# placrosse/Zaru

Hardware: AMD Instinct MI355X
Metric: end-to-end faces/sec (detect+468-pt mesh), 1080p synthetic, 1/2/4/8 GPU (higher is better)
Workload: dtype f32

## Files before the change

include/zaru_hip.h:

```cpp
#ifndef ZARU_HIP_H
#define ZARU_HIP_H

#include <stddef.h>
#include <stdint.h>

#ifdef __cplusplus
extern "C" {
#endif

#define ZR_OK 0
#define ZR_ERR_INVALID_ARGUMENT (-1)
#define ZR_ERR_MODEL (-2)
#define ZR_ERR_DEVICE (-3)
#define ZR_ERR_SHAPE (-4)
#define ZR_ERR_INTERNAL (-5)

typedef struct zr_session zr_session;

typedef struct {
    float cx, cy, w, h, rad;
} zr_view;

typedef struct {
    const uint8_t *rgba;
// ... 41 lines not shown
    int mode;
} zr_detpost_cfg;
int zr_detect_post_async(const float *d_logits, const float *d_boxes, const float *d_anchors,
                         const float *d_letterbox, size_t n, const zr_detpost_cfg *cfg,
                         int32_t *d_count, float *d_dets, size_t dcap, float *d_records, size_t rmax,
                         uint32_t first_id, uint32_t id_stride, int32_t *d_ties, void *hip_stream);

int zr_detect_post_mapped_async(const float *d_logits, const float *d_boxes, const float *d_anchors,
                                const float *d_letterbox, size_t n, const int32_t *d_map, const int32_t *d_nframes,
                                const zr_detpost_cfg *cfg, int32_t *d_count, float *d_dets, size_t dcap,
                                int32_t *d_ties, void *hip_stream);

typedef struct {
    int tiles, tile_cap;
    int keypoints;
    float iou;
    int mode;
} zr_detmerge_cfg;
int zr_detect_merge_async(const int32_t *d_tile_count, const float *d_tile_dets, const int32_t *d_due,
                          const int32_t *d_ndue, size_t n, const zr_detmerge_cfg *cfg, int32_t *d_count,
                          float *d_dets, size_t dcap, int32_t *d_ties, int32_t *d_tile_dropped, void *hip_stream);

int zr_embed_match_async(const float *d_query, size_t q, const float *d_gallery, size_t g, size_t dim,
                         const int32_t *d_valid, int32_t *d_best_idx, float *d_best_dist,
                         float *d_dist , void *hip_stream);
int zr_embed_match_count_async(const float *d_query, size_t q, const float *d_gallery, size_t g_cap,
                               const int32_t *d_g, size_t dim, const int32_t *d_valid, int32_t *d_best_idx,
                               float *d_best_dist, void *hip_stream);

typedef struct zr_comm zr_comm;
int zr_comm_unique_id(uint8_t id[128]);
int zr_comm_create(const uint8_t id[128], int nranks, int rank, int device, zr_comm **out);
void zr_comm_destroy(zr_comm *c);
int zr_comm_size(const zr_comm *c, int *nranks);
int zr_comm_all_gather_async(zr_comm *c, const void *d_send, void *d_recv, size_t bytes, void *hip_stream);

typedef struct {
    float roi[5];
    float view_rect[5];
    float local[3];
    uint32_t active;
    uint32_t frame_w, frame_h;
    uint32_t tracked;
    float confidence;
    float updated[5];
} zr_track_state;

typedef struct {
    float half_w, half_h, tl_x, tl_y, view_w, view_h, cos_r, sin_r;
    uint32_t frame, pad;
} zr_view_desc;

typedef struct {
    int kind;
    int num_landmarks;
    int in_w, in_h;
    int aspect_w, aspect_h;
    float loss_thresh, padding;
    int rois_per_frame;
} zr_track_cfg;

int zr_track_seed_async(zr_track_state *d_state, size_t n, const zr_track_cfg *cfg,
                        zr_view_desc *d_views, void *hip_stream);
int zr_track_update_async(zr_track_state *d_state, size_t n, const zr_track_cfg *cfg,
                          const float *d_landmarks, size_t lm_stride, const float *d_flag,
                          size_t flag_stride, float *d_lm_out, zr_view_desc *d_views, void *hip_stream);
int zr_track_update_indexed_async(zr_track_state *d_state, size_t n, const zr_track_cfg *cfg,
                                  const float *d_landmarks, size_t lm_stride, const float *d_flag,
                                  size_t flag_stride, const int32_t *d_index, float *d_lm_out,
                                  zr_view_desc *d_views, void *hip_stream);

enum { ZR_LM_FILTER_NONE = 0, ZR_LM_FILTER_EMA = 1, ZR_LM_FILTER_ALPHA_BETA = 2, ZR_LM_FILTER_ONE_EURO = 3 };
typedef struct {
    int kind;
    float p[3];
} zr_lm_filter;
int zr_lm_filter_state_size(const zr_lm_filter *filter, size_t num_landmarks, size_t *bytes);
int zr_lm_filter_async(const zr_lm_filter *filter, const zr_track_cfg *cfg, const zr_track_state *d_state,
                       size_t n, const float *d_landmarks, size_t lm_stride, const float *d_flag,
                       size_t flag_stride, float elapsed_s, void *d_filter_state, float *d_positions,
                       void *hip_stream);
int zr_track_update_positions_async(zr_track_state *d_state, size_t n, const zr_track_cfg *cfg,
                                    const float *d_positions, const float *d_flag, size_t flag_stride,
                                    float *d_lm_out, zr_view_desc *d_views, void *hip_stream);
int zr_lm_filter_indexed_async(const zr_lm_filter *filter, const zr_track_cfg *cfg,
                               const zr_track_state *d_state, size_t n, size_t slots,
                               const float *d_landmarks, size_t lm_stride, const float *d_flag,
                               size_t flag_stride, const int32_t *d_index, const int32_t *d_src,
                               float elapsed_s, const void *d_filter_state_in, void *d_filter_state_out,
                               float *d_positions, void *hip_stream);
int zr_track_update_positions_indexed_async(zr_track_state *d_state, size_t n, const zr_track_cfg *cfg,
                                            const float *d_positions, const float *d_flag,
                                            size_t flag_stride, const int32_t *d_index, float *d_lm_out,
                                            zr_view_desc *d_views, void *hip_stream);

typedef struct zr_procrustes zr_procrustes;
#define ZR_PROCRUSTES_MAX_POINTS 2048
int zr_procrustes_create(const float *ref_xyz, size_t n_ref, zr_procrustes **out);
void zr_procrustes_destroy(zr_procrustes *p);
typedef struct {
    float centroid[3];
    float scale;
    float translation[3];
    uint32_t valid;
    float quat[4];
    float rot[9];
} zr_pose;
int zr_procrustes_analyze_async(const zr_procrustes *p, const float *d_points, size_t n_sets, size_t stride,
                                int flip_y, const int32_t *d_valid, zr_pose *d_out, void *hip_stream);
int zr_procrustes_analyze_tracked_async(const zr_procrustes *p, const float *d_points, size_t n_sets,
                                        size_t stride, int flip_y, const zr_track_state *d_state,
                                        zr_pose *d_out, void *hip_stream);

int zr_view_describe(const zr_view *views, size_t n, uint32_t frame, zr_view_desc *out);
int zr_track_seed_detections_async(const int32_t *d_count, const float *d_dets, size_t dcap,
                                   const float *d_forced, const int32_t *d_nforced,
                                   const uint32_t *d_frame_size, size_t n, const zr_track_cfg *cfg,
                                   float roi_grow, int roi_use_angle, zr_track_state *d_state,
                                   zr_track_state *d_seed_copy, zr_view_desc *d_views, void *hip_stream);
typedef struct {
    int slots;
    float iou_thresh;
    float palm_grow;
    double interval_ms;
    int aspect_w, aspect_h;
} zr_hand_cfg;
int zr_hand_manage_async(zr_track_state *d_state, uint64_t *d_ids, float *d_hroi, int32_t *d_src,
                         int32_t *d_nhands, uint64_t *d_next_id, double *d_next_det, int32_t *d_det_pending,
                         const int32_t *d_count, const float *d_dets, size_t dcap,
                         const uint32_t *d_frame_size, size_t n, const zr_hand_cfg *cfg, double now_ms,
                         int init_clock, zr_view_desc *d_views, int32_t *d_dropped, void *hip_stream);
typedef struct {
    int slots;
    float iou_thresh;
    float det_grow;
    int use_angle;
    double interval_ms;
    int aspect_w, aspect_h;
} zr_multi_cfg;
int zr_multi_manage_async(zr_track_state *d_state, uint64_t *d_ids, float *d_roi, int32_t *d_src,
                          int32_t *d_nobjects, uint64_t *d_next_id, double *d_next_det, int32_t *d_det_pending,
                          const int32_t *d_count, const float *d_dets, size_t dcap,
                          const uint32_t *d_frame_size, size_t n, const zr_multi_cfg *cfg, double now_ms,
                          int init_clock, zr_view_desc *d_views, int32_t *d_dropped, void *hip_stream);
int zr_slot_compact_async(const int32_t *d_counts, size_t n_streams, size_t slots, const zr_view_desc *d_views,
                          zr_view_desc *d_dense_views, int32_t *d_dense_of, int32_t *d_nactive,
                          uint64_t *d_total, void *hip_stream);
int zr_cnn_estimate_device_views_async(zr_session *s, const zr_frame *frames, size_t n_frames,
                                       const zr_view_desc *d_views, size_t n_views, float lo,
                                       float hi, float *const *d_outputs, void *hip_stream);
int zr_cnn_estimate_device_views_count_async(zr_session *s, const zr_frame *frames, size_t n_frames,
                                             const zr_view_desc *d_views, size_t n_views, const int32_t *d_count,
                                             float lo, float hi, float *const *d_outputs, void *hip_stream);
int zr_due_compact_async(const int32_t *d_det_pending, size_t n, const zr_view_desc *view_template, int32_t *d_due,
                         int32_t *d_ndue, zr_view_desc *d_due_views, uint64_t *d_total, void *hip_stream);
int zr_due_compact_tiles_async(const int32_t *d_det_pending, size_t n, const zr_view_desc *d_tile_templates,
                               size_t tiles, int32_t *d_due, int32_t *d_ndue, int32_t *d_due_slots,
                               zr_view_desc *d_due_views, int32_t *d_nviews, uint64_t *d_total_streams,
                               uint64_t *d_total_views, void *hip_stream);
int zr_track_lost_compact_async(const zr_track_state *d_state, size_t n, const zr_view_desc *view_template,
                                int32_t *d_due, int32_t *d_ndue, zr_view_desc *d_due_views, uint64_t *d_total,
                                void *hip_stream);
int zr_track_reseed_best_async(const int32_t *d_count, const float *d_dets, size_t dcap, const uint32_t *d_frame_size,
                               size_t n, const zr_track_cfg *cfg, zr_track_state *d_state, zr_view_desc *d_views,
                               uint64_t *d_reseeded, void *hip_stream);

typedef struct {
    int32_t row;
    float distance;
    uint32_t embeddings;
    uint32_t flags;
    double next_ms;
} zr_identity_state;
#define ZR_IDENTITY_DIM 128
#define ZR_IDENTITY_EVER_KNOWN 1u
#define ZR_IDENTITY_ENROLLED 2u
typedef struct {
    int slots;
    int num_landmarks;
    int aspect_w, aspect_h;
    float crop_grow;
    float threshold;
    double interval_ms;
} zr_identity_cfg;
int zr_identity_select_async(const zr_identity_cfg *cfg, const zr_track_state *d_state, size_t n,
                             const float *d_landmarks, const int32_t *d_src, double now_ms,
                             const zr_identity_state *d_in, const float *d_emb_in, zr_identity_state *d_out,
                             float *d_emb_out, int32_t *d_due, zr_view_desc *d_views, void *hip_stream);
int zr_identity_compact_async(const int32_t *d_due, const zr_view_desc *d_views, size_t n,
                              zr_view_desc *d_due_views, int32_t *d_due_of, int32_t *d_ndue,
                              int32_t *d_due_valid, uint64_t *d_total, void *hip_stream);
int zr_identity_commit_async(const zr_identity_cfg *cfg, size_t n, const int32_t *d_due_of,
                             const int32_t *d_best_idx, const float *d_best_dist, const float *d_dense_emb,
                             double now_ms, zr_identity_state *d_out, float *d_emb_out, void *hip_stream);
int zr_identity_enrol_async(const zr_identity_cfg *cfg, size_t n, const int32_t *d_due_of, zr_identity_state *d_out,
                            const float *d_emb_out, float *d_gallery, uint64_t *d_ids, int32_t *d_count,
                            uint64_t *d_next_id, size_t capacity, size_t dim, uint32_t min_embeddings,
                            uint64_t *d_enrolled_total, uint64_t *d_dropped, void *hip_stream);
int zr_identity_blend_async(const zr_identity_cfg *cfg, size_t n, const int32_t *d_due_of,
                            const zr_identity_state *d_state_out, const float *d_emb_out, const float *d_dense_emb,
                            uint32_t template_cap, float *d_query, void *hip_stream);
int zr_identity_refine_async(const zr_identity_cfg *cfg, size_t n, const int32_t *d_due_of,
                             const zr_identity_state *d_state_out, const float *d_dense_emb, float *d_gallery,
                             uint32_t *d_updates, const int32_t *d_count, size_t capacity, size_t dim,
                             uint32_t max_samples, float update_threshold, uint64_t *d_refined_total,
                             void *hip_stream);
typedef struct {
    int32_t alias;
    int32_t partner;
    uint32_t seen;
    uint32_t reserved;
} zr_gallery_link;
int zr_identity_link_async(const zr_identity_cfg *cfg, const zr_track_state *d_state, size_t n,
                           const int32_t *d_src, const int32_t *d_due_of, const zr_identity_state *d_in,
                           zr_identity_state *d_out, zr_gallery_link *d_links, const int32_t *d_count,
                           size_t capacity, uint32_t min_observations, float link_threshold, uint64_t *d_counts,
                           void *hip_stream);

typedef struct {
    float size, inside, sharpness, frontal;
    uint32_t flags;
    uint32_t rejected;
    uint32_t samples;
    uint32_t reserved;
} zr_face_quality;
#define ZR_QUALITY_MEASURED 1u
#define ZR_QUALITY_EMBED 2u
#define ZR_QUALITY_LEARN 4u
#define ZR_QUALITY_FAIL_SIZE 16u
#define ZR_QUALITY_FAIL_INSIDE 32u
#define ZR_QUALITY_FAIL_SHARPNESS 64u
#define ZR_QUALITY_FAIL_FRONTAL 128u
#define ZR_QUALITY_MAX_PIXELS 16384
typedef struct {
    float min_size, min_inside, min_sharpness, min_frontal;
} zr_quality_tier;
typedef struct {
    int slots;
    int ow, oh;
    zr_quality_tier embed, learn;
} zr_quality_cfg;
int zr_identity_quality_async(const zr_quality_cfg *cfg, const zr_frame *frames, size_t n_frames,
                              const zr_track_state *d_state, size_t n, const int32_t *d_src,
                              const zr_view_desc *d_views, const zr_pose *d_pose, const zr_face_quality *d_in,
                              zr_face_quality *d_out, int32_t *d_due, uint64_t *d_measured_total,
                              uint64_t *d_rejected_total, void *hip_stream);
int zr_identity_quality_mask_async(size_t n, const int32_t *d_due_of, const zr_face_quality *d_quality,
                                   int32_t *d_due_of_learn, uint64_t *d_held_total, void *hip_stream);
int zr_face_quality_host(const zr_quality_cfg *cfg, const zr_frame *frame, const zr_view_desc *view,
                         const zr_pose *pose, zr_face_quality *out);

typedef struct {
    int32_t num_points;
    int32_t ow, oh;
    float tmpl[8][2];
    int32_t group[8][4];
    float max_residual;
} zr_align_cfg;
typedef struct {
    float scale;
    float rad;
    float residual;
    uint32_t flags;
} zr_face_alignment;
#define ZR_ALIGN_ALIGNED 1u
#define ZR_ALIGN_FALLBACK 2u
#define ZR_ALIGN_FAIL_DEGENERATE 16u
#define ZR_ALIGN_FAIL_RESIDUAL 32u
int zr_identity_align_async(const zr_align_cfg *cfg, const zr_track_state *d_state, size_t n,
                            const float *d_landmarks, size_t num_landmarks, const int32_t *d_due,
                            zr_view_desc *d_views, zr_face_alignment *d_records, uint64_t *d_totals,
                            void *hip_stream);
int zr_face_align_host(const zr_align_cfg *cfg, const float *landmarks, size_t num_landmarks, size_t stride,
                       uint32_t frame_w, uint32_t frame_h, uint32_t frame, zr_view_desc *view,
                       zr_face_alignment *out);

typedef struct {
    int slots;
    int num_landmarks;
    int aspect_w, aspect_h;
    int in_w, in_h;
    float crop_grow;
} zr_eye_cfg;
#define ZR_EYE_POINTS 76
int zr_eye_select_async(const zr_eye_cfg *cfg, const zr_track_state *d_state, size_t n, const float *d_landmarks,
                        int32_t *d_valid, zr_view_desc *d_views, float *d_crop_rect, void *hip_stream);
int zr_eye_crop_async(const zr_frame *frames, size_t n_frames, const zr_view_desc *d_due_views,
                      const int32_t *d_due_of, size_t n_entries, const int32_t *d_count, uint8_t *d_atlas,
                      uint32_t in_w, uint32_t in_h, void *hip_stream);
int zr_eye_commit_async(const zr_eye_cfg *cfg, size_t n, const int32_t *d_due_of, const float *d_out0,
                        const float *d_out1, size_t stride0, size_t stride1, const float *d_crop_rect,
                        float *d_eye_lm, float *d_eye_diam, int32_t *d_eye_valid, void *hip_stream);

#define ZR_EXPORT_POSE 1u
#define ZR_EXPORT_IDENTITY 2u
#define ZR_EXPORT_EYE_LEFT 4u
#define ZR_EXPORT_EYE_RIGHT 8u
#define ZR_EXPORT_QUALITY 16u
typedef struct {
    uint64_t id;
    int32_t stream;
    int32_t slot;
    float roi[5];
    float confidence;
    uint32_t flags;
    uint32_t reserved;
// ... 96 lines not shown
```

zaru_amd/_lib.py:

```python
from __future__ import annotations

import ctypes as C
import os

HERE = os.path.dirname(os.path.abspath(__file__))
LIB_DIR = os.path.join(HERE, "lib")
LIB_PATH = os.path.join(LIB_DIR, "libzaru_hip.so")
HEADER = os.path.join(os.path.dirname(HERE), "include", "zaru_hip.h")

ZR_OK = 0
ERRORS = {-1: "invalid argument", -2: "model", -3: "device", -4: "shape", -5: "internal"}


class ZaruError(RuntimeError):
    def __init__(self, code: int, msg: str):
        super().__init__(f"{ERRORS.get(code, code)} error: {msg}")
        self.code = code


class View(C.Structure):
    _fields_ = [("cx", C.c_float), ("cy", C.c_float), ("w", C.c_float), ("h", C.c_float),
                ("rad", C.c_float)]


# ... 51 lines not shown


class IdentityCfg(C.Structure):
    _fields_ = [("slots", C.c_int), ("num_landmarks", C.c_int), ("aspect_w", C.c_int), ("aspect_h", C.c_int),
                ("crop_grow", C.c_float), ("threshold", C.c_float), ("interval_ms", C.c_double)]


class EyeCfg(C.Structure):
    _fields_ = [("slots", C.c_int), ("num_landmarks", C.c_int), ("aspect_w", C.c_int), ("aspect_h", C.c_int),
                ("in_w", C.c_int), ("in_h", C.c_int), ("crop_grow", C.c_float)]


class FaceQuality(C.Structure):
    _fields_ = [("size", C.c_float), ("inside", C.c_float), ("sharpness", C.c_float), ("frontal", C.c_float),
                ("flags", C.c_uint32), ("rejected", C.c_uint32), ("samples", C.c_uint32), ("reserved", C.c_uint32)]


class QualityTier(C.Structure):
    _fields_ = [("min_size", C.c_float), ("min_inside", C.c_float), ("min_sharpness", C.c_float),
                ("min_frontal", C.c_float)]


class QualityCfg(C.Structure):
    _fields_ = [("slots", C.c_int), ("ow", C.c_int), ("oh", C.c_int), ("embed", QualityTier), ("learn", QualityTier)]


QUALITY_MEASURED, QUALITY_EMBED, QUALITY_LEARN = 1, 2, 4
QUALITY_FAIL_SIZE, QUALITY_FAIL_INSIDE, QUALITY_FAIL_SHARPNESS, QUALITY_FAIL_FRONTAL = 16, 32, 64, 128


class AlignCfg(C.Structure):
    _fields_ = [("num_points", C.c_int32), ("ow", C.c_int32), ("oh", C.c_int32), ("tmpl", C.c_float * 2 * 8),
                ("group", C.c_int32 * 4 * 8), ("max_residual", C.c_float)]

    @classmethod
    def make(cls, template, groups, ow=112, oh=112, max_residual=float("inf")):
        c = cls(len(template), ow, oh)
        c.max_residual = max_residual
        for p in range(8):
            for j in range(4):
                c.group[p][j] = -1
        for p, (t, g) in enumerate(zip(template[:8], groups[:8])):
            c.tmpl[p][0], c.tmpl[p][1] = float(t[0]), float(t[1])
            for j, idx in enumerate(list(g)[:4]):
                c.group[p][j] = int(idx)
        return c


class FaceAlignment(C.Structure):
    _fields_ = [("scale", C.c_float), ("rad", C.c_float), ("residual", C.c_float), ("flags", C.c_uint32)]


ALIGN_ALIGNED, ALIGN_FALLBACK, ALIGN_FAIL_DEGENERATE, ALIGN_FAIL_RESIDUAL = 1, 2, 16, 32


class ExportHeader(C.Structure):
    _fields_ = [("id", C.c_uint64), ("stream", C.c_int32), ("slot", C.c_int32), ("roi", C.c_float * 5),
                ("confidence", C.c_float), ("flags", C.c_uint32), ("reserved", C.c_uint32)]


class ExportIdentity(C.Structure):
    _fields_ = [("row", C.c_int32), ("distance", C.c_float), ("embeddings", C.c_uint32), ("flags", C.c_uint32)]


EXPORT_POSE, EXPORT_IDENTITY, EXPORT_EYE_LEFT, EXPORT_EYE_RIGHT, EXPORT_QUALITY = 1, 2, 4, 8, 16


class MultiExportArgs(C.Structure):
    INPUTS = ("d_nobjects", "d_src", "d_ids", "d_roi", "d_state", "d_landmarks")
    POSE = ("d_pose", "d_out_pose")
    IDENTITY = ("d_id_state", "d_id_emb", "d_out_identity", "d_out_emb")
    EYES = ("d_eye_valid", "d_eye_diam", "d_eye_crop", "d_eye_lm", "d_out_eye_valid", "d_out_eye_diam",
            "d_out_eye_crop", "d_out_eye_lm")
    _fields_ = [(n, C.c_void_p) for n in (
        "d_nobjects", "d_src", "d_ids", "d_roi", "d_state", "d_landmarks", "d_pose", "d_id_state", "d_id_emb",
        "d_eye_valid", "d_eye_diam", "d_eye_crop", "d_eye_lm", "d_count", "d_stream_offsets", "d_header",
        "d_out_landmarks", "d_out_pose", "d_out_identity", "d_out_emb", "d_out_eye_valid", "d_out_eye_diam",
        "d_out_eye_crop", "d_out_eye_lm")]


def lm_filter_state_size(f: LmFilter, num_landmarks: int) -> int:
    n = C.c_size_t(0)
    check(lib().zr_lm_filter_state_size(C.byref(f), num_landmarks, C.byref(n)))
    return n.value


_LIB = None

_P, _SZ, _F, _U32, _I = C.c_void_p, C.c_size_t, C.c_float, C.c_uint32, C.c_int
SIGNATURES = [
    ("zr_session_create", _I, [_P, _SZ, _P, _SZ, _I, C.POINTER(_P)]),
    ("zr_session_destroy", None, [_P]),
    ("zr_session_num_io", _I, [_P, _I, C.POINTER(_SZ)]),
    ("zr_session_io", _I, [_P, _I, _SZ, C.POINTER(C.c_char_p), _P, C.POINTER(_SZ)]),
    ("zr_session_run", _I, [_P, _SZ, _P, _SZ, _P, _SZ]),
    ("zr_session_run_async", _I, [_P, _SZ, _P, _P, _SZ, _P]),
    ("zr_cnn_estimate_views", _I, [_P, _P, _U32, _U32, _SZ, _P, _SZ, _F, _F, _P]),
    ("zr_cnn_estimate_views_async", _I, [_P, _P, _SZ, _P, _P, _SZ, _F, _F, _P, _P]),
    ("zr_preprocess_views_async", _I, [_P, _SZ, _P, _P, _SZ, _U32, _U32, _F, _F, _P, _P]),
    ("zr_detection_candidates_async", _I, [_P, _P, _U32, _U32, _U32, _F, _U32, _P, _P, _P]),
    ("zr_track_seed_async", _I, [_P, _SZ, _P, _P, _P]),
    ("zr_track_update_async", _I, [_P, _SZ, _P, _P, _SZ, _P, _SZ, _P, _P, _P]),
    ("zr_lm_filter_state_size", _I, [_P, _SZ, C.POINTER(_SZ)]),
    ("zr_lm_filter_async", _I, [_P, _P, _P, _SZ, _P, _SZ, _P, _SZ, _F, _P, _P, _P]),
    ("zr_track_update_positions_async", _I, [_P, _SZ, _P, _P, _P, _SZ, _P, _P, _P]),
    ("zr_lm_filter_indexed_async", _I, [_P, _P, _P, _SZ, _SZ, _P, _SZ, _P, _SZ, _P, _P, _F, _P, _P, _P, _P]),
    ("zr_track_update_positions_indexed_async", _I, [_P, _SZ, _P, _P, _P, _SZ, _P, _P, _P, _P]),
    ("zr_procrustes_create", _I, [_P, _SZ, C.POINTER(_P)]),
    ("zr_procrustes_destroy", None, [_P]),
    ("zr_procrustes_analyze_async", _I, [_P, _P, _SZ, _SZ, _I, _P, _P, _P]),
    ("zr_procrustes_analyze_tracked_async", _I, [_P, _P, _SZ, _SZ, _I, _P, _P, _P]),
    ("zr_view_describe", _I, [_P, _SZ, _U32, _P]),
    ("zr_detect_post_async", _I, [_P, _P, _P, _P, _SZ, _P, _P, _P, _SZ, _P, _SZ, _U32, _U32, _P, _P]),
    ("zr_detect_post_mapped_async", _I, [_P, _P, _P, _P, _SZ, _P, _P, _P, _P, _P, _SZ, _P, _P]),
    ("zr_due_compact_async", _I, [_P, _SZ, _P, _P, _P, _P, _P, _P]),
    ("zr_due_compact_tiles_async", _I, [_P, _SZ, _P, _SZ, _P, _P, _P, _P, _P, _P, _P, _P]),
    ("zr_detect_merge_async", _I, [_P, _P, _P, _P, _SZ, _P, _P, _P, _SZ, _P, _P, _P]),
    ("zr_track_lost_compact_async", _I, [_P, _SZ, _P, _P, _P, _P, _P, _P]),
    ("zr_track_reseed_best_async", _I, [_P, _P, _SZ, _P, _SZ, _P, _P, _P, _P, _P]),
    ("zr_cnn_estimate_device_views_count_async", _I, [_P, _P, _SZ, _P, _SZ, _P, _F, _F, _P, _P]),
    ("zr_track_seed_detections_async", _I, [_P, _P, _SZ, _P, _P, _P, _SZ, _P, _F, _I, _P, _P, _P, _P]),
    ("zr_hand_manage_async", _I, [_P, _P, _P, _P, _P, _P, _P, _P, _P, _P, _SZ, _P, _SZ, _P, C.c_double, _I,
                                  _P, _P, _P]),
    ("zr_multi_manage_async", _I, [_P, _P, _P, _P, _P, _P, _P, _P, _P, _P, _SZ, _P, _SZ, _P, C.c_double, _I,
                                   _P, _P, _P]),
    ("zr_slot_compact_async", _I, [_P, _SZ, _SZ, _P, _P, _P, _P, _P, _P]),
    ("zr_track_update_indexed_async", _I, [_P, _SZ, _P, _P, _SZ, _P, _SZ, _P, _P, _P, _P]),
    ("zr_embed_match_async", _I, [_P, _SZ, _P, _SZ, _SZ, _P, _P, _P, _P, _P]),
    ("zr_identity_select_async", _I, [_P, _P, _SZ, _P, _P, C.c_double, _P, _P, _P, _P, _P, _P, _P]),
    ("zr_identity_compact_async", _I, [_P, _P, _SZ, _P, _P, _P, _P, _P, _P]),
    ("zr_identity_commit_async", _I, [_P, _SZ, _P, _P, _P, _P, C.c_double, _P, _P, _P]),
    ("zr_identity_enrol_async", _I, [_P, _SZ, _P, _P, _P, _P, _P, _P, _P, _SZ, _SZ, _U32, _P, _P, _P]),
    ("zr_identity_link_async", _I, [_P, _P, _SZ, _P, _P, _P, _P, _P, _P, _SZ, _U32, C.c_float, _P, _P]),
    ("zr_identity_blend_async", _I, [_P, _SZ, _P, _P, _P, _P, _U32, _P, _P]),
    ("zr_identity_refine_async", _I, [_P, _SZ, _P, _P, _P, _P, _P, _P, _SZ, _SZ, _U32, C.c_float, _P, _P]),
    ("zr_identity_quality_async", _I, [_P, _P, _SZ, _P, _SZ, _P, _P, _P, _P, _P, _P, _P, _P, _P]),
    ("zr_identity_quality_mask_async", _I, [_SZ, _P, _P, _P, _P, _P]),
    ("zr_face_quality_host", _I, [_P, _P, _P, _P, _P]),
    ("zr_identity_align_async", _I, [_P, _P, _SZ, _P, _SZ, _P, _P, _P, _P, _P]),
    ("zr_face_align_host", _I, [_P, _P, _SZ, _SZ, _U32, _U32, _U32, _P, _P]),
    ("zr_embed_match_count_async", _I, [_P, _SZ, _P, _SZ, _P, _SZ, _P, _P, _P, _P]),
    ("zr_eye_select_async", _I, [_P, _P, _SZ, _P, _P, _P, _P, _P]),
    ("zr_eye_crop_async", _I, [_P, _SZ, _P, _P, _SZ, _P, _P, _U32, _U32, _P]),
    ("zr_eye_commit_async", _I, [_P, _SZ, _P, _P, _P, _SZ, _SZ, _P, _P, _P, _P, _P]),
    ("zr_multi_export_async", _I, [_P, _SZ, _SZ, _SZ, _P]),
    ("zr_multi_export_quality_async", _I, [_P, _P, _P, _SZ, _SZ, _SZ, _P]),
    ("zr_comm_unique_id", _I, [_P]),
    ("zr_comm_create", _I, [_P, _I, _I, _I, C.POINTER(_P)]),
    ("zr_comm_destroy", None, [_P]),
    ("zr_comm_size", _I, [_P, C.POINTER(_I)]),
    ("zr_comm_all_gather_async", _I, [_P, _P, _P, _SZ, _P]),
    ("zr_debug_glibc_math", _I, [_I, _P, _P, _P, _SZ, _P]),
    ("zr_cnn_estimate_device_views_async", _I, [_P, _P, _SZ, _P, _SZ, _F, _F, _P, _P]),
    ("zr_jpeg_decoder_create", _I, [C.c_int, _P]),
    ("zr_jpeg_decoder_destroy", None, [_P]),
    ("zr_jpeg_info", _I, [_P, _SZ, _P, _P]),
    ("zr_jpeg_decode_async", _I, [_P, _P, _SZ, _P, _SZ, _P]),
    ("zr_jpeg_decode_batch_async", _I, [_P, _SZ, _P, _P, _P, _P, _P]),
    ("zr_jpeg_coefficients", _I, [_P, _SZ, _P, _SZ, _P]),
    ("zr_jpeg_decoder_status", _I, [_P, C.POINTER(C.c_uint64), C.POINTER(C.c_uint64), C.POINTER(_I)]),
    ("zr_jpeg_frame_errors", _I, [_P, _P, _SZ, C.POINTER(_SZ)]),
    ("zr_session_stats", _I, [_P, C.POINTER(C.c_double), C.POINTER(C.c_double), C.POINTER(_SZ)]),
    ("zr_plan_describe", _I, [_P, _SZ, _P, _SZ, _P, _SZ, C.POINTER(_SZ)]),
    ("zr_profile_enable", _I, [_P, _I]),
    ("zr_profile_read", _I, [_P, _P, _SZ, C.POINTER(_SZ)]),
    ("zr_last_error", C.c_char_p, []),
    ("zr_device_count", _I, [C.POINTER(_I)]),
    ("zr_malloc", _I, [C.POINTER(_P), _SZ]),
    ("zr_free", _I, [_P]),
    ("zr_host_alloc", _I, [C.POINTER(_P), _SZ]),
    ("zr_host_free", _I, [_P]),
    ("zr_memcpy_async", _I, [_P, _P, _SZ, _I, _P]),
    ("zr_memset_async", _I, [_P, _I, _SZ, _P]),
    ("zr_memcpy2d_async", _I, [_P, _SZ, _P, _SZ, _SZ, _SZ, _I, _P]),
    ("zr_stream_create", _I, [C.POINTER(_P)]),
    ("zr_stream_destroy", _I, [_P]),
    ("zr_stream_synchronize", _I, [_P]),
    ("zr_event_create", _I, [C.POINTER(_P)]),
    ("zr_event_create_timing", _I, [C.POINTER(_P)]),
    ("zr_event_elapsed", _I, [C.POINTER(_F), _P, _P]),
    ("zr_stream_wait_event", _I, [_P, _P]),
    ("zr_event_destroy", _I, [_P]),
    ("zr_event_record", _I, [_P, _P]),
    ("zr_event_synchronize", _I, [_P]),
    ("zr_event_query", _I, [_P]),
]


def lib():
    global _LIB
    if _LIB is not None:
        return _LIB
    if not os.path.exists(LIB_PATH):
        raise ZaruError(-3, f"HIP extension not built: {LIB_PATH} missing "
                            "(run __graft_entry__.build())")
    L = C.CDLL(LIB_PATH)
    for name, res, args in SIGNATURES:
        fn = getattr(L, name)
        fn.restype = res
        fn.argtypes = args
    _LIB = L
    return L


def check(rc: int):
    if rc != ZR_OK:
        raise ZaruError(rc, lib().zr_last_error().decode(errors="replace"))


def device_count() -> int:
    n = C.c_int(0)
    check(lib().zr_device_count(C.byref(n)))
    return n.value


def plan_describe(onnx: bytes, outputs=None) -> str:
    sel = (C.c_uint32 * len(outputs))(*outputs) if outputs else None
    need = C.c_size_t(0)
    check(lib().zr_plan_describe(onnx, len(onnx), sel, len(outputs or []), None, 0,
                                 C.byref(need)))
    buf = C.create_string_buffer(need.value)
    check(lib().zr_plan_describe(onnx, len(onnx), sel, len(outputs or []), buf, need.value,
                                 C.byref(need)))
    return buf.value.decode()


class DeviceBuffer:

    def __init__(self, nbytes: int):
        p = C.c_void_p()
        check(lib().zr_malloc(C.byref(p), max(4, int(nbytes))))
        self.ptr = p.value
        self.nbytes = int(nbytes)

    @classmethod
    def from_array(cls, a, stream=None):
        import numpy as np
        a = np.ascontiguousarray(a)
        b = cls(a.nbytes)
        b.upload(a, stream)
        return b

    def upload(self, a, stream=None):
        import numpy as np
        a = np.ascontiguousarray(a)
        check(lib().zr_memcpy_async(self.ptr, a.ctypes.data, a.nbytes, 0, stream))
        check(lib().zr_stream_synchronize(stream))

    def download(self, shape, dtype, stream=None):
        import numpy as np
        out = np.empty(shape, dtype)
        check(lib().zr_memcpy_async(out.ctypes.data, self.ptr, out.nbytes, 1, stream))
        check(lib().zr_stream_synchronize(stream))
        return out

    def free(self):
        if getattr(self, "ptr", None) and _LIB is not None:
            _LIB.zr_free(self.ptr)
            self.ptr = None

    def __del__(self):
        self.free()


class Procrustes:

    def __init__(self, reference):
        import numpy as np
        ref = np.ascontiguousarray(reference, np.float32)
        if ref.ndim != 2 or ref.shape[1] != 3:
            raise ZaruError(-4, "reference must be (n, 3) float32")
        p = C.c_void_p()
        check(lib().zr_procrustes_create(ref.ctypes.data, ref.shape[0], C.byref(p)))
        self.ptr, self.n_ref = p.value, ref.shape[0]

    def analyze_async(self, d_points: int, n_sets: int, d_out: int, stride=None, flip_y=False, d_valid=None,
                      stream=None):
        check(lib().zr_procrustes_analyze_async(self.ptr, d_points, n_sets,
                                                3 * self.n_ref if stride is None else stride,
                                                int(bool(flip_y)), d_valid, d_out, stream))

    def analyze(self, points, flip_y=False, valid=None):
        import numpy as np
        pts = np.ascontiguousarray(points, np.float32)
        if pts.ndim != 3 or pts.shape[2] != 3:
            raise ZaruError(-4, "points must be (n_sets, m, 3) float32")
        d_pts = DeviceBuffer.from_array(pts)
        d_valid = None if valid is None else DeviceBuffer.from_array(np.ascontiguousarray(valid, np.int32))
        d_out = DeviceBuffer(pts.shape[0] * C.sizeof(Pose))
        self.analyze_async(d_pts.ptr, pts.shape[0], d_out.ptr, 3 * pts.shape[1], flip_y,
                           None if d_valid is None else d_valid.ptr)
        return d_out.download((pts.shape[0],), np.dtype(Pose))

    def close(self):
        if getattr(self, "ptr", None) and _LIB is not None:
            _LIB.zr_procrustes_destroy(self.ptr)
            self.ptr = None

    def __del__(self):
        self.close()


def synchronize(stream=None):
    check(lib().zr_stream_synchronize(stream))


# ... 49 lines not shown
```

zaru_amd/csrc/host/bindings.cpp:

```cpp
#include <pybind11/numpy.h>
#include <pybind11/pybind11.h>
#include <pybind11/stl.h>

#include "detection.h"
#include "hand_tracker.h"
#include "device_hand_tracker.h"
#include "device_multi_tracker.h"
#include "landmark.h"
#include "pipeline.h"
#include "procrustes.h"
#include "recognition.h"
#include "device_face_loop.h"
#include "device_tracker.h"
#include "eye.h"

namespace py = pybind11;
using namespace zh;

namespace {

Image host_image(const py::array_t<uint8_t, py::array::c_style> &a) {
    if (a.ndim() != 3 || a.shape(2) != 4) throw ZaruError(ZR_ERR_INVALID_ARGUMENT, "image must be HxWx4 uint8 RGBA");
    Image im;
    im.rgba = a.data();
// ... 718 lines not shown
        })
        .def("objects", [](DeviceMultiTracker &t, size_t s) {
            py::list out;
            for (auto &o : t.objects(s)) {
                py::dict d;
                d["id"] = o.id;
                d["landmarks"] = f32_array(o.landmarks.data(), {(py::ssize_t)(o.landmarks.size() / 3), (py::ssize_t)3});
                d["view_rect"] = o.view_rect;
                d["confidence"] = o.confidence;
                if (o.pose) d["pose"] = f32_array(reinterpret_cast<const float *>(&*o.pose), {21});
                d["identity"] = py::none();
                if (o.identity) {
                    py::dict id;
                    id["id"] = o.identity->id;
                    id["distance"] = o.identity->distance;
                    id["embeddings"] = o.identity->embeddings;
                    id["embedding"] = f32_array(o.identity->embedding.data(), {(py::ssize_t)EMBEDDING_DIM});
                    id["enrolled"] = o.identity->enrolled;
                    d["identity"] = id;
                }
                d["eyes"] = py::none();
                if (o.eyes) {
                    py::dict eyes;
                    for (int side = 0; side < 2; side++) {
                        const auto &e = side ? o.eyes->right : o.eyes->left;
                        py::object v = py::none();
                        if (e) {
                            py::dict ed;
                            ed["landmarks"] = f32_array(e->landmarks.data(), {(py::ssize_t)EYE_POINTS, (py::ssize_t)3});
                            ed["iris_diameter"] = e->iris_diameter;
                            ed["crop"] = e->crop;
                            v = ed;
                        }
                        eyes[side ? "right" : "left"] = v;
                    }
                    d["eyes"] = eyes;
                }
                if (o.quality) d["quality"] = quality_dict(*o.quality);
                out.append(d);
            }
            return out;
        });
    py::class_<DeviceTracker>(m, "DeviceTracker")
        .def(py::init([](const std::string &net, int device, float padding, float loss) {
                 return new DeviceTracker(landmark_net(net), device, padding, loss);
             }), py::arg("network") = "facemesh", py::arg("device") = 0,
             py::arg("padding") = LandmarkTracker::DEFAULT_ROI_PADDING,
             py::arg("loss_threshold") = LandmarkTracker::DEFAULT_LOSS_THRESHOLD)
        .def("set_rois", [](DeviceTracker &t, const std::vector<std::tuple<float, float, float, float, float>> &rois,
                            const std::vector<std::pair<uint32_t, uint32_t>> &sizes) {
            std::vector<RotatedRect> r;
            for (auto &v : rois)
                r.emplace_back(Rect::from_center(std::get<0>(v), std::get<1>(v), std::get<2>(v), std::get<3>(v)),
                               std::get<4>(v));
            t.set_rois(r, sizes);
        })
        .def("step", [](DeviceTracker &t, const std::vector<std::tuple<uint64_t, uint32_t, uint32_t, uint64_t>> &frames,
                        std::optional<float> elapsed) {
            const std::vector<Image> im = device_frames(frames);
            py::gil_scoped_release nogil;
            t.step(im, elapsed);
        }, py::arg("frames"), py::arg("elapsed") = py::none())
        .def("set_filter", [](DeviceTracker &t, const py::object &f, float dt) { t.set_filter(filter_arg(f), dt); },
             py::arg("filter"), py::arg("dt") = Estimator::DEFAULT_FILTER_DT)
        .def("set_pose_reference", [](DeviceTracker &t, const py::object &points, bool flip_y) {
            t.set_pose_reference(pose_reference_arg(points), flip_y);
        }, py::arg("points"), py::arg("flip_y") = true)
        .def("poses", [](DeviceTracker &t) { return poses_array(t.poses()); })
        .def("synchronize", &DeviceTracker::synchronize, py::call_guard<py::gil_scoped_release>())
        .def("__len__", &DeviceTracker::size)
        .def("states", [](DeviceTracker &t) {
            py::list out;
            for (const auto &s : t.states()) {
                py::dict d;
                d["roi"] = RotatedRect(Rect::from_center(s.roi[0], s.roi[1], s.roi[2], s.roi[3]), s.roi[4]);
                d["updated_roi"] = RotatedRect(Rect::from_center(s.updated[0], s.updated[1], s.updated[2], s.updated[3]), s.updated[4]);
                d["view_rect"] = RotatedRect(Rect::from_center(s.view_rect[0], s.view_rect[1], s.view_rect[2], s.view_rect[3]), s.view_rect[4]);
                d["active"] = s.active != 0;
                d["tracked"] = s.tracked != 0;
                d["confidence"] = s.confidence;
                out.append(d);
            }
            return out;
        })
        .def("views", [](DeviceTracker &t) {
            auto v = t.views();
            py::array_t<float> a({(py::ssize_t)v.size(), (py::ssize_t)10});
            static_assert(sizeof(zr_view_desc) == 40, "zr_view_desc");
            std::memcpy(a.mutable_data(), v.data(), v.size() * sizeof(zr_view_desc));
            return a;
        })
        .def("host_view", [](const DeviceTracker &t, const RotatedRect &roi, uint32_t fw, uint32_t fh, uint32_t frame) {
            const zr_view_desc d = t.host_view(roi, fw, fh, frame);
            py::array_t<float> a(10);
            std::memcpy(a.mutable_data(), &d, sizeof(d));
            return a;
        })
        .def("landmarks", [](DeviceTracker &t) {
            auto v = t.landmarks();
            py::array_t<float> a({(py::ssize_t)t.size(), (py::ssize_t)t.network().num_landmarks, (py::ssize_t)3});
            std::memcpy(a.mutable_data(), v.data(), v.size() * 4);
            return a;
        });

    py::class_<DeviceFaceLoop>(m, "DeviceFaceLoop")
        .def(py::init([](const std::string &detector, const std::string &landmarker, size_t streams, int device,
                         float padding, float loss, float det_threshold) {
                 return new DeviceFaceLoop(detector_net(detector), landmark_net(landmarker), streams, device, padding,
                                           loss, det_threshold);
             }), py::arg("detector") = "face", py::arg("landmarker") = "facemesh_v2", py::arg("streams") = 1,
             py::arg("device") = 0, py::arg("padding") = LandmarkTracker::DEFAULT_ROI_PADDING,
             py::arg("loss_threshold") = LandmarkTracker::DEFAULT_LOSS_THRESHOLD,
             py::arg("det_threshold") = Detector::DEFAULT_THRESHOLD)
        .def("set_roi", &DeviceFaceLoop::set_roi)
        .def("step", [](DeviceFaceLoop &t, const std::vector<std::tuple<uint64_t, uint32_t, uint32_t, uint64_t>> &frames,
                        std::optional<float> elapsed) {
            const std::vector<Image> im = device_frames(frames);
            py::gil_scoped_release nogil;
            t.step(im, elapsed);
        }, py::arg("frames"), py::arg("elapsed") = py::none())
        .def("set_filter", [](DeviceFaceLoop &t, const py::object &f, float dt) { t.set_filter(filter_arg(f), dt); },
             py::arg("filter"), py::arg("dt") = Estimator::DEFAULT_FILTER_DT)
        .def("set_pose_reference", [](DeviceFaceLoop &t, const py::object &points, bool flip_y) {
            t.set_pose_reference(pose_reference_arg(points), flip_y);
        }, py::arg("points"), py::arg("flip_y") = true)
        .def("poses", [](DeviceFaceLoop &t) { return poses_array(t.poses()); })
        .def("synchronize", &DeviceFaceLoop::synchronize, py::call_guard<py::gil_scoped_release>())
        .def("__len__", &DeviceFaceLoop::streams)
        .def("states", [](DeviceFaceLoop &t) {
            py::list out;
            for (const auto &s : t.states()) {
                py::dict d;
                d["roi"] = RotatedRect(Rect::from_center(s.roi[0], s.roi[1], s.roi[2], s.roi[3]), s.roi[4]);
                d["updated_roi"] = RotatedRect(Rect::from_center(s.updated[0], s.updated[1], s.updated[2], s.updated[3]), s.updated[4]);
                d["view_rect"] = RotatedRect(Rect::from_center(s.view_rect[0], s.view_rect[1], s.view_rect[2], s.view_rect[3]), s.view_rect[4]);
                d["active"] = s.active != 0;
                d["tracked"] = s.tracked != 0;
                d["confidence"] = s.confidence;
                out.append(d);
            }
            return out;
        })
        .def("landmarks", [](DeviceFaceLoop &t) {
            auto v = t.landmarks();
            py::array_t<float> a({(py::ssize_t)t.streams(), (py::ssize_t)t.landmarker().num_landmarks, (py::ssize_t)3});
            std::memcpy(a.mutable_data(), v.data(), v.size() * 4);
            return a;
        })
        .def("detected", &DeviceFaceLoop::detected)
        .def("detection_counts", &DeviceFaceLoop::detection_counts)
        .def("detections_run", &DeviceFaceLoop::detections_run)
        .def("reacquisitions", &DeviceFaceLoop::reacquisitions);

    py::class_<DetectTrackPipeline>(m, "DetectTrackPipeline")
        .def(py::init([](const std::string &kind, int device, int threads, uint32_t max_rois,
                         uint32_t sub_batches, bool stream_per_sub_batch, float loss_threshold,
                         const std::string &detector, const std::string &landmarker, bool device_post,
                         const std::string &nms_mode, uint32_t det_cap, float det_threshold) {
                 PipelineConfig c = kind == "hand" ? PipelineConfig::hand() : PipelineConfig::face();
                 if (kind != "hand" && kind != "face")
                     throw ZaruError(ZR_ERR_INVALID_ARGUMENT, "pipeline kind must be 'face' or 'hand'");
                 if (!detector.empty()) c.detector = detector_net(detector);
                 if (!landmarker.empty()) c.landmarker = landmark_net(landmarker);
                 c.max_rois_per_frame = max_rois;
                 c.sub_batches = sub_batches;
                 c.stream_per_sub_batch = stream_per_sub_batch;
                 c.loss_threshold = loss_threshold;
                 c.device_post = device_post;
                 if (nms_mode == "remove") c.nms_mode = SuppressionMode::Remove;
                 else if (nms_mode != "average") throw ZaruError(ZR_ERR_INVALID_ARGUMENT, "nms_mode: average | remove");
                 c.det_cap = det_cap;
                 c.det_threshold = det_threshold;
                 return new DetectTrackPipeline(c, device, threads);
             }), py::arg("kind") = "face", py::arg("device") = 0, py::arg("threads") = 8,
             py::arg("max_rois_per_frame") = 8, py::arg("sub_batches") = 2,
             py::arg("stream_per_sub_batch") = true,
             py::arg("loss_threshold") = LandmarkTracker::DEFAULT_LOSS_THRESHOLD,
             py::arg("detector") = "", py::arg("landmarker") = "", py::arg("device_post") = true,
             py::arg("nms_mode") = "average", py::arg("det_cap") = 0,
             py::arg("det_threshold") = Detector::DEFAULT_THRESHOLD)
        .def("run", [](DetectTrackPipeline &p, const std::vector<std::tuple<uint64_t, uint32_t, uint32_t, uint64_t>> &frames,
                       const std::vector<std::vector<std::tuple<float, float, float, float, float>>> &forced) {
            std::vector<Image> im;
            for (auto &f : frames) {
                Image i;
                i.rgba = reinterpret_cast<const uint8_t *>(std::get<0>(f));
                i.width = std::get<1>(f);
                i.height = std::get<2>(f);
                i.row_stride = std::get<3>(f);
                i.on_device = true;
                im.push_back(i);
            }
            std::vector<std::vector<RotatedRect>> fr(forced.size());
            for (size_t k = 0; k < forced.size(); k++)
                for (auto &t : forced[k])
                    fr[k].push_back(RotatedRect(Rect::from_center(std::get<0>(t), std::get<1>(t), std::get<2>(t), std::get<3>(t)), std::get<4>(t)));
            py::gil_scoped_release nogil;
            p.run(im, fr);
        })
        .def("set_frames", [](DetectTrackPipeline &p, const std::vector<std::tuple<uint64_t, uint32_t, uint32_t, uint64_t>> &frames,
                              const std::vector<std::vector<std::tuple<float, float, float, float, float>>> &forced) {
            std::vector<Image> im;
            for (auto &f : frames) {
                Image i;
                i.rgba = reinterpret_cast<const uint8_t *>(std::get<0>(f));
                i.width = std::get<1>(f);
                i.height = std::get<2>(f);
                i.row_stride = std::get<3>(f);
                i.on_device = true;
                im.push_back(i);
            }
            std::vector<std::vector<RotatedRect>> fr(forced.size());
            for (size_t k = 0; k < forced.size(); k++)
                for (auto &t : forced[k])
                    fr[k].push_back(RotatedRect(Rect::from_center(std::get<0>(t), std::get<1>(t), std::get<2>(t), std::get<3>(t)), std::get<4>(t)));
            p.set_frames(std::move(im), std::move(fr));
        })
        .def("run_frames", [](DetectTrackPipeline &p) {
            py::gil_scoped_release nogil;
            p.run_frames();
            return p.rois().size();
        })
        .def("run_frames_repeated", [](DetectTrackPipeline &p, int steps) {
            py::gil_scoped_release nogil;
            p.run_frames_repeated(steps);
            return p.times().tracked;
        }, py::arg("steps"))
        .def("begin_steps", [](DetectTrackPipeline &p) {
            py::gil_scoped_release nogil;
            p.begin_steps();
        })
        .def("step", [](DetectTrackPipeline &p, bool more) {
            py::gil_scoped_release nogil;
            p.step(more);
            return p.times().tracked;
        }, py::arg("more"))
        .def("detections", [](const DetectTrackPipeline &p) { return p.detections(); })
        .def("detection_records", [](const DetectTrackPipeline &p, uint32_t rmax, uint32_t first_id,
                                     uint32_t id_stride) {
            const auto &d = p.detections();
            std::vector<uint32_t> ids(d.size());
            for (size_t i = 0; i < d.size(); i++) ids[i] = first_id + (uint32_t)i * id_stride;
            py::array_t<float> a({(py::ssize_t)d.size(), (py::ssize_t)det_record_width(rmax)});
            pack_detection_records(d, ids, rmax, a.mutable_data());
            return a;
        }, py::arg("rmax") = 8, py::arg("first_id") = 0, py::arg("id_stride") = 1)
        .def("enable_records", [](DetectTrackPipeline &p, uint32_t rmax, uint32_t first_id, uint32_t id_stride,
                                  uint64_t comm, int world) {
            p.enable_records(rmax, first_id, id_stride, reinterpret_cast<zr_comm *>(comm), world);
        }, py::arg("rmax") = 8, py::arg("first_id") = 0, py::arg("id_stride") = 1, py::arg("comm") = 0,
           py::arg("world") = 1)
        .def("records", [](DetectTrackPipeline &p) {
            std::vector<float> r;
            {
                py::gil_scoped_release nogil;
                r = p.records();
            }
            const py::ssize_t w = p.record_width();
            py::array_t<float> a({(py::ssize_t)r.size() / w, w});
            std::memcpy(a.mutable_data(), r.data(), r.size() * 4);
            return a;
        })
        .def("gathered", [](DetectTrackPipeline &p) {
            std::vector<float> r;
            {
                py::gil_scoped_release nogil;
                r = p.gathered();
            }
            const py::ssize_t w = p.record_width();
            py::array_t<float> a({(py::ssize_t)r.size() / w, w});
            std::memcpy(a.mutable_data(), r.data(), r.size() * 4);
            return a;
        })
        .def("num_rois", [](const DetectTrackPipeline &p) { return p.rois().size(); })
        .def("roi", [](const DetectTrackPipeline &p, size_t i) {
            const RoiResult &r = p.rois().at(i);
            py::dict d = estimate_dict(r.result.estimate);
            d["frame"] = r.frame;
            d["from_detection"] = r.from_detection;
            d["tracked"] = r.tracked;
            d["confidence"] = r.confidence;
            d["roi"] = r.roi;
            d["view_rect"] = r.result.view_rect;
            d["updated_roi"] = r.result.updated_roi;
            d["next_roi"] = r.next_roi;
            return d;
        })
        .def("times", [](const DetectTrackPipeline &p) {
            const StageTimes &t = p.times();
            py::dict d;
            d["detect_gpu_ms"] = t.detect_gpu_ms;
            d["decode_nms_ms"] = t.decode_nms_ms;
            d["landmark_gpu_ms"] = t.landmark_gpu_ms;
            d["map_ms"] = t.map_ms;
            d["total_ms"] = t.total_ms;
            d["host_wait_ms"] = t.host_wait_ms;
            d["dropped_detections"] = t.dropped_detections;
            d["nms_candidates"] = t.nms_candidates;
            d["nms_tied"] = t.nms_tied;
            d["nms_unpinned_frames"] = t.nms_unpinned_frames;
            d["frames"] = t.frames;
            d["detections"] = t.detections;
            d["rois"] = t.rois;
            d["tracked"] = t.tracked;
            return d;
        })
        .def("stats", [](const DetectTrackPipeline &p) {
            py::dict d;
            d["detector_bytes_per_image"] = p.detector_bytes_per_image();
            d["landmarker_bytes_per_image"] = p.landmarker_bytes_per_image();
            d["detector_flops_per_image"] = p.detector_flops_per_image();
            d["landmarker_flops_per_image"] = p.landmarker_flops_per_image();
            return d;
        })
        .def("stream", [](const DetectTrackPipeline &p) { return reinterpret_cast<uint64_t>(p.stream()); })
        .def("profile", &DetectTrackPipeline::profile)
        .def("profile_read", &DetectTrackPipeline::profile_read);

    auto model_vec = [](const py::bytes &b) {
        const std::string s = b;
        return std::vector<uint8_t>(s.begin(), s.end());
    };
    auto embedding_of = [](const py::array_t<float, py::array::c_style> &a) {
        if ((size_t)a.size() != EMBEDDING_DIM) throw ZaruError(ZR_ERR_SHAPE, "an embedding is 128 floats");
        Embedding e;
        std::memcpy(e.v.data(), a.data(), EMBEDDING_DIM * sizeof(float));
        return e;
    };
    auto embedding_array = [](const Embedding &e) {
        py::array_t<float> a((py::ssize_t)EMBEDDING_DIM);
        std::memcpy(a.mutable_data(), e.v.data(), EMBEDDING_DIM * sizeof(float));
        return a;
    };
    auto device_frames = [](const std::vector<std::tuple<uint64_t, uint32_t, uint32_t, uint64_t>> &frames) {
        std::vector<Image> im;
        for (auto &f : frames) {
            Image i;
            i.rgba = reinterpret_cast<const uint8_t *>(std::get<0>(f));
            i.width = std::get<1>(f);
            i.height = std::get<2>(f);
            i.row_stride = std::get<3>(f);
            i.on_device = true;
            im.push_back(i);
        }
        return im;
    };
    m.attr("NO_MATCH") = NO_MATCH;
    py::class_<Embedding>(m, "Embedding")
        .def(py::init(embedding_of))
        .def("difference", &Embedding::difference)
        .def("values", embedding_array);
    py::class_<FaceEmbedder>(m, "FaceEmbedder")
        .def(py::init([model_vec](const py::bytes &model, int device) { return new FaceEmbedder(model_vec(model), device); }),
             py::arg("model"), py::arg("device") = 0)
        .def("input_width", [](const FaceEmbedder &e) { return e.cnn().input_width(); })
        .def("session", [](const FaceEmbedder &e) { return reinterpret_cast<uint64_t>(e.cnn().nn().handle()); })
        .def("crop_view", &FaceEmbedder::crop_view)
        .def("embed", [](const FaceEmbedder &e, py::array_t<uint8_t, py::array::c_style> img, const std::vector<Rect> &rects) {
            const auto v = e.embed(host_image(img), rects);
            py::array_t<float> a({(py::ssize_t)v.size(), (py::ssize_t)EMBEDDING_DIM});
            for (size_t i = 0; i < v.size(); i++)
                std::memcpy(a.mutable_data() + i * EMBEDDING_DIM, v[i].v.data(), EMBEDDING_DIM * sizeof(float));
            return a;
        })
        .def("embed_views", [](const FaceEmbedder &e, py::array_t<uint8_t, py::array::c_style> img,
                               const std::vector<ViewData> &views) {
            const auto v = e.embed_views(host_image(img), views);
            py::array_t<float> a({(py::ssize_t)v.size(), (py::ssize_t)EMBEDDING_DIM});
            for (size_t i = 0; i < v.size(); i++)
                std::memcpy(a.mutable_data() + i * EMBEDDING_DIM, v[i].v.data(), EMBEDDING_DIM * sizeof(float));
            return a;
        })
        .def("embed_first_face", [embedding_array](const FaceEmbedder &e, Detector &d,
                                                   py::array_t<uint8_t, py::array::c_style> img) -> py::object {
            Embedding out;
            if (!e.embed_first_face(d, host_image(img), out)) return py::none();
            return embedding_array(out);
        });
    m.def("landmark_crop_view", [](py::array_t<float, py::array::c_style> landmarks, uint32_t image_w, uint32_t image_h,
                                   uint32_t aspect_w, uint32_t aspect_h, float grow) {
        if (landmarks.ndim() != 2 || landmarks.shape(0) < 1 || landmarks.shape(1) < 2)
            throw ZaruError(ZR_ERR_SHAPE, "landmarks must be [L >= 1][C >= 2]");
        return landmark_crop_view(landmarks.data(), (size_t)landmarks.shape(0), image_w, image_h, aspect_w, aspect_h,
                                  grow, (size_t)landmarks.shape(1));
    }, py::arg("landmarks"), py::arg("image_w"), py::arg("image_h"), py::arg("aspect_w"), py::arg("aspect_h"),
          py::arg("grow") = FaceEmbedder::CROP_GROW);
    m.def("aligned_crop_view", [](py::array_t<float, py::array::c_style> landmarks, uint32_t image_w, uint32_t image_h,
                                  const FaceAlignment &alignment) {
        if (landmarks.ndim() != 2 || landmarks.shape(0) < 1 || landmarks.shape(1) < 2)
            throw ZaruError(ZR_ERR_SHAPE, "landmarks must be [L >= 1][C >= 2]");
        zr_face_alignment r{};
        const auto v = aligned_crop_view(landmarks.data(), (size_t)landmarks.shape(0), image_w, image_h, alignment,
                                         (size_t)landmarks.shape(1), &r);
        py::dict d;
        d["scale"] = r.scale;
        d["angle"] = r.rad;
        d["residual"] = r.residual;
        d["flags"] = r.flags;
        return py::make_tuple(v ? py::cast(*v) : py::object(py::none()), d);
    }, py::arg("landmarks"), py::arg("image_w"), py::arg("image_h"), py::arg("alignment"));
    auto face_mesh_arg = [](const py::array_t<float, py::array::c_style | py::array::forcecast> &lm) {
        if (lm.ndim() != 2 || lm.shape(0) < 387 || lm.shape(1) != 3)
            throw ZaruError(ZR_ERR_SHAPE, "face landmarks must be (L >= 387, 3) float32");
    };
    auto refined_eye = [](const std::optional<RefinedEye> &e) -> py::object {
        if (!e) return py::none();
        py::dict d;
        d["landmarks"] = f32_array(e->landmarks.positions().data(), {(py::ssize_t)EYE_POINTS, (py::ssize_t)3});
        d["iris_diameter"] = e->iris_diameter;
        d["crop"] = e->crop;
        return d;
    };
    m.attr("EYE_CROP_GROW") = EYE_CROP_GROW;
    m.def("face_eye_rects", [face_mesh_arg](py::array_t<float, py::array::c_style | py::array::forcecast> lm) {
        face_mesh_arg(lm);
        const EyeRects r = face_eye_rects(lm.data(), (size_t)lm.shape(0), 3);
        return py::make_tuple(r.left ? py::cast(*r.left) : py::object(py::none()),
                              r.right ? py::cast(*r.right) : py::object(py::none()));
    }, py::arg("landmarks"));
    m.def("eye_crop_rect", [](const RotatedRect &r, float grow) { return eye_crop_rect(r, grow); }, py::arg("rect"),
          py::arg("grow") = EYE_CROP_GROW);
    m.def("eye_crop_view", [](const RotatedRect &r, uint32_t w, uint32_t h, float grow) {
        return eye_crop_view(r, w, h, grow);
    }, py::arg("rect"), py::arg("image_w"), py::arg("image_h"), py::arg("grow") = EYE_CROP_GROW);
    m.def("eye_map_out", [refined_eye](py::array_t<float, py::array::c_style | py::array::forcecast> raw, bool right,
                                       const RotatedRect &crop) {
        if (raw.ndim() != 2 || raw.shape(0) != (py::ssize_t)EYE_POINTS || raw.shape(1) != 3)
            throw ZaruError(ZR_ERR_SHAPE, "eye landmarks are (76, 3) float32");
        return refined_eye(eye_map_out(raw.data(), right, crop));
    }, py::arg("raw"), py::arg("right"), py::arg("crop"));
    py::class_<EyeLandmarks>(m, "EyeLandmarks")
        .def(py::init([](py::array_t<float, py::array::c_style | py::array::forcecast> p) {
                 if (p.ndim() != 2 || p.shape(0) != (py::ssize_t)EYE_POINTS || p.shape(1) != 3)
                     throw ZaruError(ZR_ERR_SHAPE, "eye landmarks are (76, 3) float32");
                 return new EyeLandmarks(p.data());
             }), py::arg("positions"))
        .def("positions", [](const EyeLandmarks &e) { return f32_array(e.positions().data(), {(py::ssize_t)EYE_POINTS, 3}); })
        .def("iris_center", [](const EyeLandmarks &e) { return f32_array(e.iris_center().data(), {3}); })
        .def("iris_contour", [](const EyeLandmarks &e) { return f32_array(e.iris_contour().data(), {4, 3}); })
        .def("eye_contour", [](const EyeLandmarks &e) { return f32_array(e.eye_contour().data(), {(py::ssize_t)EYE_POINTS - 5, 3}); })
        .def("iris_diameter", &EyeLandmarks::iris_diameter)
        .def("flip_horizontal_in_place", &EyeLandmarks::flip_horizontal_in_place, py::arg("width"));
    py::class_<EyeRefiner>(m, "EyeRefiner")
        .def(py::init<int>(), py::arg("device") = 0)
        .def("input_width", &EyeRefiner::input_width)
        .def("refine", [face_mesh_arg, refined_eye](EyeRefiner &r, py::array_t<uint8_t, py::array::c_style> img,
                                                   py::array_t<float, py::array::c_style | py::array::forcecast> lm, float grow) {
            face_mesh_arg(lm);
            const RefinedEyes e = r.refine(host_image(img), lm.data(), (size_t)lm.shape(0), grow);
// ... 125 lines not shown
```

zaru_amd/csrc/host/pipeline.cpp:

```cpp
#include "pipeline.h"

#include <algorithm>
#include <condition_variable>
#include <cstring>
#include <mutex>

namespace zh {

struct ThreadPool::Impl {
    std::mutex mu;
    std::condition_variable cv, done_cv;
    const std::function<void(size_t)> *fn = nullptr;
    size_t n = 0;
    std::atomic<size_t> next{0};
    uint64_t generation = 0;
    int busy = 0;
    bool stop = false;

    void work() {
        for (;;) {
            size_t i = next.fetch_add(1);
            if (i >= n) break;
            (*fn)(i);
        }
    }
};

ThreadPool::ThreadPool(int n) : impl_(new Impl) {
    for (int t = 1; t < std::max(1, n); t++)
        workers_.emplace_back([this] {
            Impl &I = *impl_;
            uint64_t seen = 0;
            for (;;) {
                {
                    std::unique_lock<std::mutex> lk(I.mu);
                    I.cv.wait(lk, [&] { return I.stop || I.generation != seen; });
                    if (I.stop) return;
                    seen = I.generation;
                    I.busy++;
                }
                I.work();
                {
                    std::lock_guard<std::mutex> lk(I.mu);
                    if (--I.busy == 0) I.done_cv.notify_all();
                }
            }
        });
}

ThreadPool::~ThreadPool() {
    {
        std::lock_guard<std::mutex> lk(impl_->mu);
        impl_->stop = true;
    }
    impl_->cv.notify_all();
    for (auto &t : workers_) t.join();
}

void ThreadPool::parallel_for(size_t n, const std::function<void(size_t)> &fn) {
    if (n == 0) return;
    Impl &I = *impl_;
    if (workers_.empty() || n == 1) {
        for (size_t i = 0; i < n; i++) fn(i);
        return;
    }
    {
        std::lock_guard<std::mutex> lk(I.mu);
        I.fn = &fn;
        I.n = n;
        I.next = 0;
        I.generation++;
    }
    I.cv.notify_all();
    I.work();
    std::unique_lock<std::mutex> lk(I.mu);
    I.done_cv.wait(lk, [&] { return I.busy == 0 && I.next.load() >= I.n; });
    I.fn = nullptr;
}

PipelineConfig PipelineConfig::face() {
    PipelineConfig c;
    c.detector = DetectorNetwork::short_range_face();
    c.landmarker = LandmarkNetwork::face_mesh_v1();
    c.roi_grow = 0.f;
    c.roi_use_angle = false;
    c.roi_padding = LandmarkTracker::DEFAULT_ROI_PADDING;
    return c;
}

PipelineConfig PipelineConfig::hand() {
    PipelineConfig c;
    c.detector = DetectorNetwork::palm_lite();
    c.landmarker = LandmarkNetwork::hand_lite();
    c.roi_grow = 1.5f;
    c.roi_use_angle = true;
    c.roi_padding = 0.4f;
    return c;
}

DetectTrackPipeline::DetectTrackPipeline(PipelineConfig cfg, int device, int threads)
    : cfg_(std::move(cfg)), device_(device), det_cnn_(network_cnn(cfg_.detector.kind, device)),
      lm_cnn_(network_cnn(cfg_.landmarker.kind, device)), pool_(threads) {
    nms_.set_iou_thresh(cfg_.nms_iou);
    nms_.set_mode(cfg_.nms_mode);
    if (cfg_.device_post) {
        if (cfg_.det_cap == 0) cfg_.det_cap = (uint32_t)cfg_.detector.anchors().size();
        if (cfg_.det_cap < cfg_.max_rois_per_frame) cfg_.det_cap = cfg_.max_rois_per_frame;
        const auto &a = cfg_.detector.anchors();
        d_anchors_.resize(2 * a.size());
        check(zr_memcpy_async(d_anchors_.ptr, a.data(), a.size() * sizeof(Vec2), 0, nullptr));
        check(zr_stream_synchronize(nullptr));
    }
    check(zr_stream_create(&stream_));
    for (uint32_t i = 0; i < std::max(1u, cfg_.sub_batches); i++) {
        slots_.push_back(std::make_unique<Slot>());
        Slot &s = *slots_.back();
        if (cfg_.stream_per_sub_batch && i > 0) check(zr_stream_create(&s.stream));
        else s.stream = stream_;
        check(zr_event_create(&s.ev_det));
        check(zr_event_create(&s.ev_lm));
        check(zr_event_create(&s.ev_rec));
        for (auto &e : s.ev_t) check(zr_event_create_timing(&e));
    }
}

DetectTrackPipeline::~DetectTrackPipeline() {
    for (auto &s : slots_) {
        if (s->stream) zr_stream_synchronize(s->stream);
        if (s->stream && s->stream != stream_) zr_stream_destroy(s->stream);
        if (s->ev_det) zr_event_destroy(s->ev_det);
        if (s->ev_lm) zr_event_destroy(s->ev_lm);
        if (s->ev_rec) zr_event_destroy(s->ev_rec);
        for (auto e : s->ev_t)
            if (e) zr_event_destroy(e);
    }
    if (gstream_) {
        zr_stream_synchronize(gstream_);
        zr_stream_destroy(gstream_);
    }
    for (auto e : ev_gath_)
        if (e) zr_event_destroy(e);
    if (stream_) zr_stream_destroy(stream_);
}

size_t DetectTrackPipeline::det_cap() const { return cfg_.det_cap; }

void DetectTrackPipeline::enable_records(uint32_t rmax, uint32_t first_id, uint32_t id_stride, zr_comm *comm,
                                         int world) {
    if (!cfg_.device_post) throw ZaruError(ZR_ERR_INVALID_ARGUMENT, "device records need device post-processing");
    if (rmax == 0 || rmax > 64 || world < 1) throw ZaruError(ZR_ERR_INVALID_ARGUMENT, "bad record configuration");
    if (comm) {
        int nranks = 0;
        check(zr_comm_size(comm, &nranks));
        if (nranks != world)
            throw ZaruError(ZR_ERR_INVALID_ARGUMENT, "world (" + std::to_string(world) + ") is not the communicator's rank count (" +
                                                         std::to_string(nranks) + ")");
    }
    if (gstream_) check(zr_stream_synchronize(gstream_));
    rec_rmax_ = rmax;
    rec_first_ = first_id;
    rec_stride_ = id_stride;
    comm_ = comm;
    world_ = comm ? world : 1;
    if (!gstream_) check(zr_stream_create(&gstream_));
    for (int k = 0; k < 2; k++) {
        if (!ev_gath_[k]) check(zr_event_create(&ev_gath_[k]));
        gath_used_[k] = false;
    }
}

void DetectTrackPipeline::enqueue_gather() {
    if (!rec_rmax_) return;
    const int set = (int)(enq_steps_ & 1);
    for (size_t k = 0; k < active_slots_; k++) check(zr_stream_wait_event(gstream_, slots_[k]->ev_rec));
    if (comm_) {
        const size_t bytes = frames_.size() * record_width() * sizeof(float);
        d_gath_[set].resize((size_t)world_ * frames_.size() * record_width());
        check(zr_comm_all_gather_async(comm_, d_rec_[set].ptr, d_gath_[set].ptr, bytes, gstream_));
    }
    check(zr_event_record(ev_gath_[set], gstream_));
    gath_used_[set] = true;
    enq_steps_++;
}

std::vector<float> DetectTrackPipeline::records() {
    if (!rec_rmax_ || done_steps_ == 0) throw ZaruError(ZR_ERR_INVALID_ARGUMENT, "no finished step with records");
    const int set = (int)((done_steps_ - 1) & 1);
    check(zr_event_synchronize(ev_gath_[set]));
    std::vector<float> out(frames_.size() * record_width());
    check(zr_memcpy_async(out.data(), d_rec_[set].ptr, out.size() * 4, 1, nullptr));
    check(zr_stream_synchronize(nullptr));
    return out;
}

std::vector<float> DetectTrackPipeline::gathered() {
    if (!comm_ || done_steps_ == 0) throw ZaruError(ZR_ERR_INVALID_ARGUMENT, "no gathered step (no communicator)");
    const int set = (int)((done_steps_ - 1) & 1);
    check(zr_event_synchronize(ev_gath_[set]));
    std::vector<float> out((size_t)world_ * frames_.size() * record_width());
    check(zr_memcpy_async(out.data(), d_gath_[set].ptr, out.size() * 4, 1, nullptr));
    check(zr_stream_synchronize(nullptr));
    return out;
}

static double session_stat(const Cnn &c, bool flops) {
    double b = 0, f = 0;
    size_t n = 0;
    check(zr_session_stats(c.nn().handle(), &b, &f, &n));
    return flops ? f : b;
}
double DetectTrackPipeline::detector_bytes_per_image() const { return session_stat(*det_cnn_, false); }
double DetectTrackPipeline::landmarker_bytes_per_image() const { return session_stat(*lm_cnn_, false); }
double DetectTrackPipeline::detector_flops_per_image() const { return session_stat(*det_cnn_, true); }
double DetectTrackPipeline::landmarker_flops_per_image() const { return session_stat(*lm_cnn_, true); }

void DetectTrackPipeline::profile(bool on) {
    check(zr_profile_enable(det_cnn_->nn().handle(), on ? 1 : 0));
    check(zr_profile_enable(lm_cnn_->nn().handle(), on ? 1 : 0));
}

std::string DetectTrackPipeline::profile_read() {
    std::string out;
    const std::pair<const char *, const Cnn *> nets[2] = {{"detector", det_cnn_.get()}, {"landmarker", lm_cnn_.get()}};
    std::vector<char> buf(1 << 16);
    for (auto &nc : nets) {
        size_t need = 0;
        check(zr_profile_read(nc.second->nn().handle(), buf.data(), buf.size(), &need));
        const std::string txt(buf.data());
        size_t pos = 0;
        while (pos < txt.size()) {
            size_t e = txt.find('\n', pos);
            if (e == std::string::npos) e = txt.size();
            if (e > pos) out += std::string(nc.first) + "/" + txt.substr(pos, e - pos) + "\n";
            pos = e + 1;
        }
    }
    return out;
}

void DetectTrackPipeline::set_frames(std::vector<Image> frames, std::vector<std::vector<RotatedRect>> forced) {
    frames_ = std::move(frames);
    forced_ = std::move(forced);
    for (auto &s : slots_) s->inputs_ok = false;
}

namespace {
using clk = std::chrono::steady_clock;
double ms_since(clk::time_point t) {
    return std::chrono::duration<double, std::milli>(clk::now() - t).count();
}
}

void DetectTrackPipeline::stage_detect(Slot &s, const std::vector<Image> &frames) {
    const Cnn &dc = *det_cnn_;
    const uint32_t A = (uint32_t)cfg_.detector.anchors().size(), D = (uint32_t)cfg_.detector.params;
    const uint32_t cap = cfg_.candidate_cap, rec_w = 2 + D;
    const size_t n = s.nf;
    s.zf.resize(n);
    s.letterbox.resize(n);
    std::vector<zr_view> zv(n);
    std::vector<uint32_t> vf(n);
    for (size_t i = 0; i < n; i++) {
        const Image &im = frames[s.f0 + i];
        if (!im.on_device) throw ZaruError(ZR_ERR_INVALID_ARGUMENT, "pipeline frames must be device-resident");
        s.zf[i] = zr_frame{im.rgba, im.width, im.height, im.row_stride};
        zv[i] = to_zr_view(letterbox_view(im.width, im.height, dc.aspect(), &s.letterbox[i]));
        vf[i] = (uint32_t)i;
    }
    s.d_boxes.resize(n * A * D);
    s.d_logits.resize(n * A);
    s.d_count.resize(n);
    s.d_rec.resize(n * cap * rec_w);
    float *douts[2] = {s.d_boxes.ptr, s.d_logits.ptr};
    if (cfg_.device_post) check(zr_event_record(s.ev_t[0], s.stream));
    dc.estimate_async(s.zf, zv, vf, douts, s.stream);
    if (cfg_.device_post) {
        check(zr_event_record(s.ev_t[1], s.stream));
        return;
    }
    check(zr_detection_candidates_async(s.d_logits.ptr, s.d_boxes.ptr, (uint32_t)n, A, D,
                                        candidate_logit_floor(cfg_.det_threshold), cap, s.d_count.ptr,
                                        s.d_rec.ptr, s.stream));
    s.h_count.resize(n);
    s.h_rec.resize(n * cap * rec_w);
    check(zr_memcpy_async(s.h_count.data(), s.d_count.ptr, n * sizeof(int32_t), 1, s.stream));
    check(zr_memcpy_async(s.h_rec.data(), s.d_rec.ptr, n * cap * rec_w * sizeof(float), 1, s.stream));
    check(zr_event_record(s.ev_det, s.stream));
}

zr_track_cfg DetectTrackPipeline::track_cfg() const {
    const Cnn &lc = *lm_cnn_;
    zr_track_cfg c{};
    c.kind = track_kind(cfg_.landmarker.kind);
    c.num_landmarks = cfg_.landmarker.num_landmarks;
    c.in_w = (int)lc.input_width();
    c.in_h = (int)lc.input_height();
    c.aspect_w = (int)lc.aspect().w;
    c.aspect_h = (int)lc.aspect().h;
    c.loss_thresh = cfg_.loss_threshold;
    c.padding = cfg_.roi_padding;
    c.rois_per_frame = (int)std::max(1u, cfg_.max_rois_per_frame);
    return c;
}

void DetectTrackPipeline::stage_device_post(Slot &s, const std::vector<Image> &frames,
                                            const std::vector<std::vector<RotatedRect>> &forced) {
    const Cnn &dc = *det_cnn_, &lc = *lm_cnn_;
    const size_t n = s.nf, R = std::max(1u, cfg_.max_rois_per_frame), dcap = cfg_.det_cap;
    const size_t nv = n * R, nout = lc.nn().num_outputs();
    const int L = cfg_.landmarker.num_landmarks;
    const uint32_t A = (uint32_t)cfg_.detector.anchors().size(), D = (uint32_t)cfg_.detector.params;
    if (!s.inputs_ok) {
        s.h_lbox.resize(4 * n);
        s.h_fsize.resize(2 * n);
        s.h_forced.resize(5 * nv);
        s.h_nforced.resize(n);
        for (size_t i = 0; i < n; i++) {
            const size_t f = s.f0 + i;
            const Rect &r = s.letterbox[i];
            s.h_lbox[4 * i] = r.center().x;
            s.h_lbox[4 * i + 1] = r.center().y;
            s.h_lbox[4 * i + 2] = r.width();
            s.h_lbox[4 * i + 3] = r.height();
            s.h_fsize[2 * i] = frames[f].width;
            s.h_fsize[2 * i + 1] = frames[f].height;
            const size_t nf = f < forced.size() ? std::min(R, forced[f].size()) : 0;
            s.h_nforced[i] = (int32_t)nf;
            for (size_t k = 0; k < nf; k++) {
                const RotatedRect &q = forced[f][k];
                float *o = &s.h_forced[5 * (i * R + k)];
                o[0] = q.rect().center().x;
                o[1] = q.rect().center().y;
                o[2] = q.rect().width();
                o[3] = q.rect().height();
                o[4] = q.rotation_radians();
            }
        }
        s.d_lbox.resize(4 * n);
        s.d_fsize.resize(2 * n);
        s.d_forced.resize(5 * nv);
        s.d_nforced.resize(n);
        check(zr_memcpy_async(s.d_lbox.ptr, s.h_lbox.ptr, 4 * n * 4, 0, s.stream));
        check(zr_memcpy_async(s.d_fsize.ptr, s.h_fsize.ptr, 2 * n * 4, 0, s.stream));
        check(zr_memcpy_async(s.d_forced.ptr, s.h_forced.ptr, 5 * nv * 4, 0, s.stream));
        check(zr_memcpy_async(s.d_nforced.ptr, s.h_nforced.ptr, n * 4, 0, s.stream));
        s.inputs_ok = true;
    }
    Slot::Results &o = s.res[s.wr];
    const size_t sum_bytes = 2 * nv * sizeof(zr_track_state) + 3 * n * sizeof(int32_t);
    o.sum.resize(sum_bytes);
    o.h_sum.resize(sum_bytes);
    o.dets.resize(n * dcap * 20);
    o.lmout.resize(nv * L * 3);
    zr_track_state *d_state = reinterpret_cast<zr_track_state *>(o.sum.ptr);
    zr_track_state *d_seed = d_state + nv;
    int32_t *d_count = reinterpret_cast<int32_t *>(d_seed + nv);
    int32_t *d_ties = d_count + n;
    s.d_views.resize(nv);
    zr_detpost_cfg pc{};
    pc.face = is_face_detector(cfg_.detector.kind) ? 1 : 0;
    pc.anchors = (int)A;
    pc.params = (int)D;
    pc.keypoints = cfg_.detector.keypoints;
    pc.in_w = (int)dc.input_width();
    pc.in_h = (int)dc.input_height();
    pc.thresh = cfg_.det_threshold;
    pc.iou = cfg_.nms_iou;
    pc.mode = cfg_.nms_mode == SuppressionMode::Remove ? 1 : 0;
    float *rec = nullptr;
    const bool records = rec_rmax_ && &frames == &frames_;
    if (records) {
        const int set = (int)(enq_steps_ & 1);
        d_rec_[set].resize(frames_.size() * record_width());
        if (gath_used_[set]) check(zr_stream_wait_event(s.stream, ev_gath_[set]));
        rec = d_rec_[set].ptr + s.f0 * record_width();
    }
    check(zr_detect_post_async(s.d_logits.ptr, s.d_boxes.ptr, d_anchors_.ptr, s.d_lbox.ptr, n, &pc, d_count,
                               o.dets.ptr, dcap, rec, rec_rmax_, rec_first_ + (uint32_t)s.f0 * rec_stride_,
                               rec_stride_, d_ties, s.stream));
    if (records) check(zr_event_record(s.ev_rec, s.stream));
    const zr_track_cfg tc = track_cfg();
    check(zr_track_seed_detections_async(d_count, o.dets.ptr, dcap, s.d_forced.ptr, s.d_nforced.ptr, s.d_fsize.ptr,
                                         n, &tc, cfg_.roi_grow, cfg_.roi_use_angle ? 1 : 0, d_state, d_seed,
                                         s.d_views.ptr, s.stream));
    check(zr_event_record(s.ev_t[2], s.stream));
    float *lptr[4] = {nullptr, nullptr, nullptr, nullptr};
    for (size_t k = 0; k < nout && k < 4; k++) {
        o.lm[k].resize((size_t)lc.nn().output_per_image(k) * nv);
        lptr[k] = o.lm[k].ptr;
    }
    const ColorMapper cm = lc.color_mapper();
    check(zr_cnn_estimate_device_views_async(lc.nn().handle(), s.zf.data(), n, s.d_views.ptr, nv, cm.lo, cm.hi, lptr,
                                             s.stream));
    check(zr_event_record(s.ev_t[3], s.stream));
    const bool flagged = tc.kind <= 2;
    check(zr_track_update_async(d_state, nv, &tc, lptr[0], (size_t)lc.nn().output_per_image(0),
                                flagged ? lptr[1] : nullptr, flagged ? (size_t)lc.nn().output_per_image(1) : 0,
                                o.lmout.ptr, s.d_views.ptr, s.stream));
    check(zr_event_record(s.ev_t[4], s.stream));
    check(zr_memcpy_async(o.h_sum.ptr, o.sum.ptr, sum_bytes, 1, s.stream));
    check(zr_event_record(s.ev_lm, s.stream));
    s.timed = true;
    s.wr ^= 1;
}

void DetectTrackPipeline::finish_device(Slot &s) {
    s.done = s.wr ^ 1;
    const Slot::Results &o = s.res[s.done];
    const size_t n = s.nf, R = std::max(1u, cfg_.max_rois_per_frame), nv = n * R;
    const zr_track_state *st = reinterpret_cast<const zr_track_state *>(o.h_sum.ptr);
    const int32_t *cnt = reinterpret_cast<const int32_t *>(st + 2 * nv), *tie = cnt + n;
    for (size_t i = 0; i < n; i++) {
        add_ties(NonMaxSuppression::TieCount{tie[2 * i], tie[2 * i + 1]});
        times_.detections += (size_t)cnt[i];
        if ((size_t)cnt[i] > cfg_.det_cap) times_.dropped_detections += (size_t)cnt[i] - cfg_.det_cap;
    }
    if (s.timed) {
        float ms[4] = {0.f, 0.f, 0.f, 0.f};
        for (int k = 0; k < 4; k++) check(zr_event_elapsed(&ms[k], s.ev_t[k], s.ev_t[k + 1]));
        times_.detect_gpu_ms += ms[0];
        times_.decode_nms_ms += ms[1];
        times_.landmark_gpu_ms += ms[2];
        times_.map_ms += ms[3];
        s.timed = false;
    }
    for (size_t v = 0; v < nv; v++) {
        times_.rois += st[nv + v].active ? 1 : 0;
        times_.tracked += st[v].tracked ? 1 : 0;
    }
    stale_ = true;
}

void DetectTrackPipeline::materialize() const {
    if (!stale_) return;
    stale_ = false;
    rois_.clear();
    for (auto &d : dets_) d.clear();
    for (size_t k = 0; k < std::min(active_slots_, slots_.size()); k++) unpack_device(*slots_[k]);
}

void DetectTrackPipeline::unpack_device(Slot &s) const {
    const Cnn &lc = *lm_cnn_;
    const size_t n = s.nf, R = std::max(1u, cfg_.max_rois_per_frame), dcap = cfg_.det_cap, nv = n * R;
    const int L = cfg_.landmarker.num_landmarks, nkp = cfg_.detector.keypoints;
    const size_t nout = lc.nn().num_outputs();
    const Slot::Results &o = s.res[s.done];
    const zr_track_state *state = reinterpret_cast<const zr_track_state *>(o.h_sum.ptr);
    const zr_track_state *seed = state + nv;
    const int32_t *count = reinterpret_cast<const int32_t *>(seed + nv);
    int maxc = 0;
    for (size_t i = 0; i < n; i++) maxc = std::max(maxc, std::min(count[i], (int32_t)dcap));
    const size_t dw = (size_t)maxc;
    std::vector<float> dets(std::max<size_t>(1, n * dw * 20)), lmout(nv * L * 3), extra[2];
    check(zr_memcpy2d_async(dets.data(), dw * 80, o.dets.ptr, dcap * 80, dw * 80, n, 1, nullptr));
    check(zr_memcpy_async(lmout.data(), o.lmout.ptr, lmout.size() * 4, 1, nullptr));
    for (size_t k = 2; k < nout && k < 4; k++) {
        extra[k - 2].resize((size_t)lc.nn().output_per_image(k) * nv);
        check(zr_memcpy_async(extra[k - 2].data(), o.lm[k].ptr, extra[k - 2].size() * 4, 1, nullptr));
    }
    check(zr_stream_synchronize(nullptr));
    for (size_t i = 0; i < n; i++) {
        const size_t f = s.f0 + i;
        const int cnt = count[i];
        auto &fd = dets_[f];
        fd.clear();
        for (int k = 0; k < cnt && k < (int)dcap; k++) {
            const float *e = &dets[(i * dw + k) * 20];
            Detection d;
            d.confidence = e[0];
            d.angle = e[1];
            d.rect = Rect::from_center(e[2], e[3], e[4], e[5]);
            for (int p = 0; p < nkp; p++) d.keypoints.push_back(Vec2{e[6 + 2 * p], e[7 + 2 * p]});
            fd.push_back(std::move(d));
        }
        for (size_t k = 0; k < R; k++) {
            const size_t v = i * R + k;
            const zr_track_state &s0 = seed[v];
            if (!s0.active) continue;
            RoiResult r;
            r.frame = (uint32_t)f;
            r.from_detection = (int)k < cnt;
            r.roi = RotatedRect(Rect::from_center(s0.roi[0], s0.roi[1], s0.roi[2], s0.roi[3]), s0.roi[4]);
            r.result.view_rect = RotatedRect(
                Rect::from_center(s0.view_rect[0], s0.view_rect[1], s0.view_rect[2], s0.view_rect[3]), s0.view_rect[4]);
            const zr_track_state &st = state[v];
            r.confidence = st.confidence;
            r.tracked = st.tracked != 0;
            if (r.tracked) {
                r.result.updated_roi = RotatedRect(
                    Rect::from_center(st.updated[0], st.updated[1], st.updated[2], st.updated[3]), st.updated[4]);
                r.next_roi = RotatedRect(Rect::from_center(st.roi[0], st.roi[1], st.roi[2], st.roi[3]), st.roi[4]);
                Estimate &e = r.result.estimate;
                const float *lm = &lmout[v * L * 3];
                e.positions.assign(lm, lm + 3 * L);
                e.confidence = st.confidence;
                if (cfg_.landmarker.kind == NetworkKind::FaceMeshV2 && nout > 2) e.tongue_out = extra[0][v];
                if (cfg_.landmarker.kind == NetworkKind::HandLandmarkLite && nout > 3) {
                    e.raw_handedness = extra[0][v];
                    const float *w = &extra[1][v * 3 * L];
                    e.world.assign(w, w + 3 * L);
                }
            }
            rois_.push_back(std::move(r));
        }
    }
}

void DetectTrackPipeline::stage_decode_and_rois(Slot &s, const std::vector<Image> &frames,
                                                const std::vector<std::vector<RotatedRect>> &forced) {
    const Cnn &dc = *det_cnn_;
    const uint32_t din_w = dc.input_width(), din_h = dc.input_height();
    const uint32_t A = (uint32_t)cfg_.detector.anchors().size(), D = (uint32_t)cfg_.detector.params;
    const uint32_t cap = cfg_.candidate_cap, rec_w = 2 + D;
    const size_t n = s.nf;
    std::vector<std::vector<float>> full_boxes(n), full_logits(n);
    bool overflow = false;
    for (size_t i = 0; i < n; i++)
        if ((uint32_t)s.h_count[i] > cap) {
            overflow = true;
            full_boxes[i].resize((size_t)A * D);
            full_logits[i].resize(A);
            check(zr_memcpy_async(full_boxes[i].data(), s.d_boxes.ptr + i * A * D, (size_t)A * D * 4, 1, s.stream));
            check(zr_memcpy_async(full_logits[i].data(), s.d_logits.ptr + i * A, (size_t)A * 4, 1, s.stream));
        }
    if (overflow) check(zr_stream_synchronize(s.stream));
    const float thresh = cfg_.det_threshold;
    pool_.parallel_for(n, [&](size_t i) {
        std::vector<Detection> raw;
        if (!full_logits[i].empty()) {
            cfg_.detector.extract(full_boxes[i].data(), full_logits[i].data(), thresh, din_w, din_h, raw);
        } else {
            const int cnt = s.h_count[i];
            const float *rec = &s.h_rec[i * cap * rec_w];
            std::vector<std::pair<uint32_t, int>> order;
            for (int k = 0; k < cnt; k++) {
                uint32_t a;
                std::memcpy(&a, &rec[k * rec_w], 4);
                order.push_back({a, k});
            }
            std::sort(order.begin(), order.end());
            for (auto &o : order) {
                const float *r = &rec[o.second * rec_w];
                const float conf = sigmoid(r[1]);
                if (conf < thresh) continue;
                raw.push_back(cfg_.detector.decode(o.first, r + 2, conf, din_w, din_h));
            }
        }
        auto &dets = dets_[s.f0 + i];
        dets = nms_.process(raw, &ties_[s.f0 + i]);
        map_detections(dets, s.letterbox[i], din_w);
    });

    const Cnn &lc = *lm_cnn_;
    const AspectRatio la = lc.aspect();
    s.rv.clear();
    s.rf.clear();
    s.local_rect.clear();
    s.roi0 = rois_.size();
    for (size_t i = 0; i < n; i++) {
        const size_t f = s.f0 + i;
        std::vector<std::pair<RotatedRect, bool>> seeds;
        for (const auto &d : dets_[f]) {
            if (seeds.size() >= cfg_.max_rois_per_frame) break;
            seeds.push_back({RotatedRect(cfg_.roi_grow > 0.f ? d.rect.grow_rel(cfg_.roi_grow) : d.rect,
                                         cfg_.roi_use_angle ? d.angle : 0.f), true});
        }
        if (seeds.empty() && f < forced.size())
            for (const auto &r : forced[f]) {
                if (seeds.size() >= cfg_.max_rois_per_frame) break;
                seeds.push_back({r, false});
            }
        const ViewData full = ViewData::full(frames[f].width, frames[f].height);
        for (const auto &sd : seeds) {
            RoiResult r;
            r.frame = (uint32_t)f;
            r.from_detection = sd.second;
            r.roi = sd.first;
            r.result.view_rect = sd.first.grow_to_fit_aspect(la);
            const ViewData view = full.view(r.result.view_rect);
            const Rect rect = view.local_rect().grow_to_fit_aspect(la);
            s.rv.push_back(to_zr_view(view.view(RotatedRect(rect, 0.f))));
            s.rf.push_back((uint32_t)i);
            s.local_rect.push_back(rect);
            rois_.push_back(r);
        }
    }
    s.nroi = rois_.size() - s.roi0;
    if (s.nroi == 0) return;
    const size_t nout = lc.nn().num_outputs();
    std::vector<float *> lptr(nout);
    for (size_t k = 0; k < nout; k++) {
        s.d_lm[k].resize((size_t)lc.nn().output_per_image(k) * s.nroi);
        lptr[k] = s.d_lm[k].ptr;
    }
    lc.estimate_async(s.zf, s.rv, s.rf, lptr.data(), s.stream);
    for (size_t k = 0; k < nout; k++) {
        const size_t cnt = (size_t)lc.nn().output_per_image(k) * s.nroi;
        s.h_lm[k].resize(cnt);
        check(zr_memcpy_async(s.h_lm[k].data(), lptr[k], cnt * 4, 1, s.stream));
    }
    check(zr_event_record(s.ev_lm, s.stream));
}

void DetectTrackPipeline::stage_map(Slot &s) {
    const Cnn &lc = *lm_cnn_;
    const uint32_t lin_w = lc.input_width();
    const size_t nout = lc.nn().num_outputs();
    pool_.parallel_for(s.nroi, [&](size_t i) {
        RoiResult &r = rois_[s.roi0 + i];
        const float *outs[4];
        for (size_t k = 0; k < nout; k++) outs[k] = &s.h_lm[k][i * lc.nn().output_per_image(k)];
        Estimate e;
        extract_landmarks(cfg_.landmarker, outs, e, lin_w, lc.input_height());
        map_estimate(e, s.local_rect[i], lin_w);
        r.confidence = e.confidence;
        r.tracked = tracker_update(cfg_.landmarker, r.roi, r.result.view_rect, cfg_.loss_threshold,
                                   cfg_.roi_padding, e, r.result, r.next_roi);
    });
}

void DetectTrackPipeline::run(const std::vector<Image> &frames,
                              const std::vector<std::vector<RotatedRect>> &forced) {
    const auto t0 = clk::now();
    const size_t B = frames.size();
    times_ = StageTimes{};
    times_.frames = B;
    dets_.assign(B, {});
    ties_.assign(B, {});
    rois_.clear();
    if (B == 0) return;
    const size_t S = std::min<size_t>(slots_.size(), B);
    size_t f0 = 0;
    for (size_t k = 0; k < S; k++) {
        Slot &s = *slots_[k];
        s.f0 = f0;
        s.nf = B / S + (k < B % S ? 1 : 0);
        f0 += s.nf;
        s.inputs_ok = false;
        stage_detect(s, frames);
        if (cfg_.device_post) stage_device_post(s, frames, forced);
    }
    active_slots_ = S;
    if (cfg_.device_post && rec_rmax_ && &frames == &frames_) enqueue_gather();
    for (size_t k = 0; k < S && cfg_.device_post; k++) {
        Slot &s = *slots_[k];
        const auto t = clk::now();
        check(zr_event_synchronize(s.ev_lm));
        times_.host_wait_ms += ms_since(t);
        finish_device(s);
    }
    if (cfg_.device_post) done_steps_ = enq_steps_;
    if (cfg_.device_post) {
        times_.total_ms = ms_since(t0);
        return;
    }
    for (size_t k = 0; k < S && !cfg_.device_post; k++) {
        Slot &s = *slots_[k];
        const auto t = clk::now();
        check(zr_event_synchronize(s.ev_det));
        times_.detect_gpu_ms += ms_since(t);
        const auto t1 = clk::now();
        stage_decode_and_rois(s, frames, forced);
        times_.decode_nms_ms += ms_since(t1);
    }
    for (size_t k = 0; k < S && !cfg_.device_post; k++) {
        Slot &s = *slots_[k];
        const auto t = clk::now();
        if (s.nroi) check(zr_event_synchronize(s.ev_lm));
        times_.landmark_gpu_ms += ms_since(t);
        const auto t1 = clk::now();
        stage_map(s);
        times_.map_ms += ms_since(t1);
    }
    times_.rois = rois_.size();
    for (auto &d : dets_) times_.detections += d.size();
    for (const auto &t : ties_) add_ties(t);
    for (auto &r : rois_) times_.tracked += r.tracked ? 1 : 0;
    times_.total_ms = ms_since(t0);
}

void DetectTrackPipeline::begin_steps() {
    steps_t0_ = clk::now();
    times_ = StageTimes{};
    if (gstream_) check(zr_stream_synchronize(gstream_));
    enq_steps_ = done_steps_ = 0;
    gath_used_[0] = gath_used_[1] = false;
    const std::vector<Image> &frames = frames_;
    const size_t B = frames.size();
    active_slots_ = std::min<size_t>(slots_.size(), B);
    size_t f0 = 0;
    for (size_t k = 0; k < active_slots_; k++) {
        Slot &s = *slots_[k];
        s.f0 = f0;
        s.nf = B / active_slots_ + (k < B % active_slots_ ? 1 : 0);
        f0 += s.nf;
        s.inputs_ok = false;
        stage_detect(s, frames);
        if (cfg_.device_post) stage_device_post(s, frames, forced_);
    }
    if (cfg_.device_post) enqueue_gather();
}

void DetectTrackPipeline::step(bool more) {
    const std::vector<Image> &frames = frames_;
    const size_t B = frames.size(), S = active_slots_;
    if (S == 0) return;
    dets_.assign(B, {});
    ties_.assign(B, {});
    rois_.clear();
    for (size_t k = 0; k < S && cfg_.device_post; k++) {
        Slot &s = *slots_[k];
        const auto t = clk::now();
        check(zr_event_synchronize(s.ev_lm));
        times_.host_wait_ms += ms_since(t);
        finish_device(s);
        if (more) {
            stage_detect(s, frames);
            stage_device_post(s, frames, forced_);
        }
    }
    if (cfg_.device_post) {
        done_steps_++;
        if (more) enqueue_gather();
        times_.frames += B;
        times_.total_ms = ms_since(steps_t0_);
        return;
    }
    for (size_t k = 0; k < S && !cfg_.device_post; k++) {
        Slot &s = *slots_[k];
        const auto t = clk::now();
        check(zr_event_synchronize(s.ev_det));
        times_.detect_gpu_ms += ms_since(t);
        const auto t1 = clk::now();
        stage_decode_and_rois(s, frames, forced_);
        times_.decode_nms_ms += ms_since(t1);
        if (more) stage_detect(s, frames);
    }
    for (size_t k = 0; k < S && !cfg_.device_post; k++) {
        Slot &s = *slots_[k];
        const auto t = clk::now();
        if (s.nroi) check(zr_event_synchronize(s.ev_lm));
        times_.landmark_gpu_ms += ms_since(t);
        const auto t1 = clk::now();
        stage_map(s);
        times_.map_ms += ms_since(t1);
    }
    times_.frames += B;
    times_.rois += rois_.size();
    for (auto &d : dets_) times_.detections += d.size();
    for (const auto &t : ties_) add_ties(t);
    for (auto &r : rois_) times_.tracked += r.tracked ? 1 : 0;
    times_.total_ms = ms_since(steps_t0_);
}

void DetectTrackPipeline::run_frames_repeated(int steps) {
    if (frames_.empty() || steps <= 0) {
        times_ = StageTimes{};
        return;
    }
    begin_steps();
    for (int it = 0; it < steps; it++) step(it + 1 < steps);
}

}
```

zaru_amd/csrc/host/pipeline.h:

```cpp
#pragma once
#include <atomic>
#include <chrono>
#include <functional>
#include <memory>
#include <thread>
#include <vector>

#include "detection.h"
#include "device_tracker.h"
#include "landmark.h"

namespace zh {

class ThreadPool {
  public:
    explicit ThreadPool(int n);
    ~ThreadPool();
    void parallel_for(size_t n, const std::function<void(size_t)> &fn);
    int size() const { return (int)workers_.size() + 1; }

  private:
    struct Impl;
    std::unique_ptr<Impl> impl_;
    std::vector<std::thread> workers_;
};

struct RoiResult {
    uint32_t frame = 0;
    bool from_detection = false;
    bool tracked = false;
    float confidence = 0.f;
    RotatedRect roi;
    TrackingResult result;
    RotatedRect next_roi;
};

struct StageTimes {
    double detect_gpu_ms = 0, decode_nms_ms = 0, landmark_gpu_ms = 0, map_ms = 0, total_ms = 0;
    double host_wait_ms = 0;
    size_t frames = 0, detections = 0, rois = 0, tracked = 0;
    size_t dropped_detections = 0;
    size_t nms_candidates = 0, nms_tied = 0, nms_unpinned_frames = 0;
};

struct PipelineConfig {
    DetectorNetwork detector = DetectorNetwork::short_range_face();
    LandmarkNetwork landmarker = LandmarkNetwork::face_mesh_v1();
    float det_threshold = Detector::DEFAULT_THRESHOLD;
    float nms_iou = NonMaxSuppression::DEFAULT_IOU_THRESH;
    SuppressionMode nms_mode = SuppressionMode::Average;
    float roi_grow = 0.f;
    bool roi_use_angle = false;
    float roi_padding = LandmarkTracker::DEFAULT_ROI_PADDING;
    float loss_threshold = LandmarkTracker::DEFAULT_LOSS_THRESHOLD;
    uint32_t max_rois_per_frame = 8;
    uint32_t candidate_cap = 64;
    uint32_t sub_batches = 2;
    bool stream_per_sub_batch = true;
    bool device_post = true;
    uint32_t det_cap = 0;
    static PipelineConfig face();
    static PipelineConfig hand();
};

class DetectTrackPipeline {
  public:
    DetectTrackPipeline(PipelineConfig cfg, int device = 0, int threads = 8);
    ~DetectTrackPipeline();

    void run(const std::vector<Image> &frames, const std::vector<std::vector<RotatedRect>> &forced);

    const std::vector<std::vector<Detection>> &detections() const {
        materialize();
        return dets_;
    }
    const std::vector<RoiResult> &rois() const {
        materialize();
        return rois_;
    }
    const StageTimes &times() const { return times_; }
    const PipelineConfig &config() const { return cfg_; }
    double detector_bytes_per_image() const;
    double landmarker_bytes_per_image() const;
    double detector_flops_per_image() const;
    double landmarker_flops_per_image() const;
    void *stream() const { return stream_; }
    void profile(bool on);
    std::string profile_read();

    void set_frames(std::vector<Image> frames, std::vector<std::vector<RotatedRect>> forced);
    void run_frames() { run(frames_, forced_); }
    void run_frames_repeated(int steps);
    void begin_steps();
    void step(bool more);

    void enable_records(uint32_t rmax, uint32_t first_id, uint32_t id_stride, zr_comm *comm = nullptr,
                        int world = 1);
    uint32_t record_width() const { return 2 + 20 * rec_rmax_; }
    std::vector<float> records();
    std::vector<float> gathered();

  private:
    struct Slot {
        size_t f0 = 0, nf = 0;
        void *stream = nullptr;
        void *ev_det = nullptr, *ev_lm = nullptr;
        void *ev_t[5] = {nullptr, nullptr, nullptr, nullptr, nullptr};
        void *ev_rec = nullptr;
        bool timed = false;
        DeviceArray<float> d_boxes, d_logits, d_rec, d_lm[4];
        DeviceArray<int32_t> d_count;
        PinnedArray<float> h_rec, h_lm[4];
        PinnedArray<int32_t> h_count;
        std::vector<zr_frame> zf;
        std::vector<Rect> letterbox, local_rect;
        std::vector<zr_view> rv;
        std::vector<uint32_t> rf;
        size_t roi0 = 0, nroi = 0;
        DeviceArray<float> d_lbox, d_forced;
        DeviceArray<uint32_t> d_fsize;
        DeviceArray<int32_t> d_nforced;
        DeviceArray<zr_view_desc> d_views;
        PinnedArray<float> h_lbox, h_forced;
        PinnedArray<uint32_t> h_fsize;
        PinnedArray<int32_t> h_nforced;
        bool inputs_ok = false;
        struct Results {
            DeviceArray<uint8_t> sum;
            DeviceArray<float> dets, lmout, lm[4];
            PinnedArray<uint8_t> h_sum;
        } res[2];
        int wr = 0;
        int done = 0;
    };
    void stage_device_post(Slot &s, const std::vector<Image> &frames,
                           const std::vector<std::vector<RotatedRect>> &forced);
    void finish_device(Slot &s);
    void unpack_device(Slot &s) const;
    void materialize() const;
    zr_track_cfg track_cfg() const;
    void stage_detect(Slot &s, const std::vector<Image> &frames);
    void stage_decode_and_rois(Slot &s, const std::vector<Image> &frames,
                               const std::vector<std::vector<RotatedRect>> &forced);
    void stage_map(Slot &s);
    void enqueue_gather();
    size_t det_cap() const;

    PipelineConfig cfg_;
    int device_;
    std::shared_ptr<const Cnn> det_cnn_, lm_cnn_;
    DeviceArray<float> d_anchors_;
    NonMaxSuppression nms_;
    ThreadPool pool_;
    void *stream_ = nullptr;
    std::vector<std::unique_ptr<Slot>> slots_;
    mutable std::vector<std::vector<Detection>> dets_;
    std::vector<NonMaxSuppression::TieCount> ties_;
    void add_ties(const NonMaxSuppression::TieCount &t) {
        times_.nms_candidates += (size_t)t.candidates;
        times_.nms_tied += (size_t)t.tied;
        times_.nms_unpinned_frames += t.unpinned() ? 1 : 0;
    }
    mutable std::vector<RoiResult> rois_;
    mutable bool stale_ = false;
    StageTimes times_;
    std::vector<Image> frames_;
    std::vector<std::vector<RotatedRect>> forced_;
    size_t active_slots_ = 0;
    std::chrono::steady_clock::time_point steps_t0_;
    uint32_t rec_rmax_ = 0, rec_first_ = 0, rec_stride_ = 1;
    zr_comm *comm_ = nullptr;
    int world_ = 1;
    DeviceArray<float> d_rec_[2], d_gath_[2];
    void *gstream_ = nullptr, *ev_gath_[2] = {nullptr, nullptr};
    bool gath_used_[2] = {false, false};
    uint64_t enq_steps_ = 0, done_steps_ = 0;
};

}
```

zaru_amd/csrc/runtime/session.cpp:

```cpp
#include <hip/hip_runtime.h>

#include <cmath>
#include <algorithm>
#include <atomic>
#include <cstdio>
#include <cstring>
#include <map>
#include <memory>
#include <mutex>
#include <string>
#include <vector>

#include "../../../include/zaru_hip.h"
#include "onnx_model.h"
#include "plan.h"
#include "zr_track.h"
#include "zr_align.h"
#include "../kernels/procrustes_math.h"
#include "../kernels/eye_math.h"
#include "../kernels/quality_math.h"

namespace {

thread_local std::string g_err;
// ... 86 lines not shown
#pragma clang fp contract(off)
    zr::ViewDesc d{};
    d.half_w = v.w * 0.5f;
    d.half_h = v.h * 0.5f;
    d.tl_x = v.cx - v.w * 0.5f;
    d.tl_y = v.cy - v.h * 0.5f;
    d.view_w = v.w;
    d.view_h = v.h;
    d.cos_r = cosf(v.rad);
    d.sin_r = sinf(v.rad);
    d.frame = frame;
    return d;
}

struct Profiler final : zr::LaunchHook {
    struct Rec {
        const char *kernel;
        double bytes, flops;
        hipEvent_t a, b;
    };
    std::mutex mu;
    std::atomic<bool> on{false};
    std::vector<Rec> recs;
    std::vector<hipEvent_t> pool;
    hipEvent_t pending = nullptr;

    hipEvent_t get() {
        if (!pool.empty()) {
            hipEvent_t e = pool.back();
            pool.pop_back();
            return e;
        }
        hipEvent_t e = nullptr;
        (void)hipEventCreate(&e);
        return e;
    }
    void before(hipStream_t s) override {
        pending = get();
        (void)hipEventRecord(pending, s);
    }
    void cancel() override {
        if (pending) pool.push_back(pending);
        pending = nullptr;
    }
    void after(hipStream_t s, const char *k, double bytes, double flops) override {
        hipEvent_t e = get();
        (void)hipEventRecord(e, s);
        recs.push_back({k, bytes, flops, pending, e});
    }
    ~Profiler() {
        for (auto &r : recs) {
            (void)hipEventDestroy(r.a);
            (void)hipEventDestroy(r.b);
        }
        for (auto e : pool) (void)hipEventDestroy(e);
    }
};

}

struct SessionRegistry {
    std::mutex mu;
    std::vector<zr_session *> live;
};
static SessionRegistry &sessions() {
    static SessionRegistry *r = new SessionRegistry;
    return *r;
}

struct zr_session {
    Profiler prof;
    int device = 0;
    zr::Plan plan;
    float *weights = nullptr;
    std::vector<std::unique_ptr<Ctx>> pool;
    std::mutex pool_mu;
    size_t next = 0;

    Ctx *acquire() {
        std::lock_guard<std::mutex> g(pool_mu);
        for (size_t i = 0; i < pool.size(); i++) {
            Ctx *c = pool[(next + i) % pool.size()].get();
            if (c->mu.try_lock()) {
                const hipError_t q = hipEventQuery(c->done);
                if (q == hipSuccess) {
                    next = (next + i + 1) % pool.size();
                    return c;
                }
                if (q != hipErrorNotReady) (void)hipGetLastError();
                c->mu.unlock();
            }
        }
        if (pool.size() < 8) {
            auto c = std::make_unique<Ctx>();
            (void)hipSetDevice(device);
            if (hipEventCreateWithFlags(&c->done, hipEventDisableTiming) != hipSuccess) return nullptr;
            c->mu.lock();
            pool.push_back(std::move(c));
            return pool.back().get();
        }
        Ctx *c = pool[next].get();
        next = (next + 1) % pool.size();
        c->mu.lock();
        (void)hipEventSynchronize(c->done);
        return c;
    }

    zr_session() {
        SessionRegistry &r = sessions();
        std::lock_guard<std::mutex> g(r.mu);
        r.live.push_back(this);
    }
    ~zr_session() {
        {
            SessionRegistry &r = sessions();
            std::lock_guard<std::mutex> g(r.mu);
            r.live.erase(std::remove(r.live.begin(), r.live.end(), this), r.live.end());
        }
        pool.clear();
        (void)hipFree(weights);
    }
};

static void forget_stream(hipStream_t stream) {
    if (!stream) return;
    SessionRegistry &r = sessions();
    std::lock_guard<std::mutex> g(r.mu);
    for (zr_session *s : r.live) {
        std::lock_guard<std::mutex> pl(s->pool_mu);
        for (auto &c : s->pool) {
            std::lock_guard<std::mutex> cl(c->mu);
            if (c->done_on != stream || !c->done) continue;
            (void)hipEventSynchronize(c->done);
            hipEvent_t fresh = nullptr;
            if (hipEventCreateWithFlags(&fresh, hipEventDisableTiming) == hipSuccess) {
                (void)hipEventDestroy(c->done);
                c->done = fresh;
            }
            c->done_on = nullptr;
        }
    }
}

namespace {

struct CtxLock {
    Ctx *c;
    explicit CtxLock(Ctx *x) : c(x) {}
    ~CtxLock() {
        if (c) c->mu.unlock();
    }
};

int enqueue(zr_session *s, Ctx *c, int N, const float *input, int64_t in_sN, int64_t in_sC,
            float *const *outs, hipStream_t stream, const zr::PreprocParams *pre = nullptr,
            const int *d_nact = nullptr) {
    const int Ns = (N + 3) / 4 * 4;
    const size_t need = (size_t)s->plan.arena_per_image * (size_t)Ns;
    size_t largest = std::max(need, (size_t)(input ? in_sN : 0) * (size_t)N);
    for (const auto &o : s->plan.outputs) largest = std::max(largest, (size_t)o.per_image * (size_t)N);
    if (largest >= ((size_t)1 << 31))
        return set_err(ZR_ERR_INVALID_ARGUMENT, "batch too large: a tensor would exceed 2^31 elements; split it");
    if (int rc = grow(c->arena, c->arena_floats, need ? need : 1)) return rc;
    HIP_TRY(hipStreamWaitEvent(stream, c->done, 0));
    zr::Binding b;
    b.N = N;
    b.Ns = Ns;
    b.input = input;
    b.in_sN = in_sN;
    b.in_sC = in_sC;
    b.outputs = outs;
    b.arena = c->arena;
    b.weights = s->weights;
    b.pre = pre;
    b.nact = d_nact;
    {
        const bool prof = s->prof.on.load();
        std::unique_lock<std::mutex> pl(s->prof.mu, std::defer_lock);
        if (prof) pl.lock();
        zr::run_plan(s->plan, b, stream, prof ? &s->prof : nullptr);
    }
    HIP_TRY(hipGetLastError());
    HIP_TRY(hipEventRecord(c->done, stream));
    c->done_on = stream;
    return ZR_OK;
}

int ctx_stream(Ctx *c) {
    if (!c->stream) HIP_TRY(hipStreamCreateWithFlags(&c->stream, hipStreamNonBlocking));
    return ZR_OK;
}

int check_session(const zr_session *s) {
    if (!s) return set_err(ZR_ERR_INVALID_ARGUMENT, "null session");
    return ZR_OK;
}

int sync_outputs(zr_session *s, Ctx *c, size_t batch) {
    const auto &po = s->plan.outputs;
    c->outs.resize(po.size(), nullptr);
    c->outs_floats.resize(po.size(), 0);
    for (size_t i = 0; i < po.size(); i++)
        if (int rc = grow(c->outs[i], c->outs_floats[i], (size_t)po[i].per_image * batch)) return rc;
    return ZR_OK;
}

int upload_views(Ctx *c, const zr_frame *frames, size_t nf, const zr_view *views,
                 const uint32_t *view_frame, size_t nv, hipStream_t stream) {
    const size_t foff = (nv * sizeof(zr::ViewDesc) + 255) & ~(size_t)255;
    const size_t bytes = foff + (nf ? nf : 1) * sizeof(zr::FrameDesc);
    if (c->desc_bytes < bytes) {
        (void)hipFree(c->desc);
        (void)hipHostFree(c->h_desc);
        c->desc = c->h_desc = nullptr;
        c->desc_bytes = 0;
        const size_t cap = bytes + bytes / 2 + 4096;
        HIP_TRY(hipMalloc((void **)&c->desc, cap));
        HIP_TRY(hipHostMalloc((void **)&c->h_desc, cap));
        c->desc_bytes = cap;
    }
    zr::ViewDesc *hv = reinterpret_cast<zr::ViewDesc *>(c->h_desc);
    zr::FrameDesc *hf = reinterpret_cast<zr::FrameDesc *>(c->h_desc + foff);
    c->views = reinterpret_cast<zr::ViewDesc *>(c->desc);
    c->frames = reinterpret_cast<zr::FrameDesc *>(c->desc + foff);
    for (size_t i = 0; i < nv; i++) {
        const uint32_t f = view_frame ? view_frame[i] : 0;
        if (f >= nf) return set_err(ZR_ERR_INVALID_ARGUMENT, "view_frame index out of range");
        hv[i] = make_view(views[i], f);
    }
    for (size_t i = 0; i < nf; i++) {
        if (!frames[i].rgba || frames[i].width == 0 || frames[i].height == 0)
            return set_err(ZR_ERR_INVALID_ARGUMENT, "empty frame");
        hf[i].rgba = frames[i].rgba;
        hf[i].w = frames[i].width;
        hf[i].h = frames[i].height;
        hf[i].stride = frames[i].row_stride;
    }
    HIP_TRY(hipMemcpyAsync(c->desc, c->h_desc, foff + nf * sizeof(zr::FrameDesc), hipMemcpyHostToDevice, stream));
    return ZR_OK;
}

}

extern "C" {

const char *zr_last_error(void) { return g_err.c_str(); }

int zr_session_create(const uint8_t *onnx, size_t len, const uint32_t *out_sel, size_t n_sel,
                      int device, zr_session **out) {
    return guarded([&]() -> int {
        if (!onnx || !out) return set_err(ZR_ERR_INVALID_ARGUMENT, "null model or out pointer");
        *out = nullptr;
        zr::OnnxModel m;
        std::string err;
        if (!zr::parse_onnx(onnx, len, m, err)) return set_err(ZR_ERR_MODEL, "ONNX parse error: " + err);
        auto s = std::make_unique<zr_session>();
        s->device = device;
        std::vector<uint32_t> sel(out_sel, out_sel + n_sel);
        if (!zr::compile_plan(m, sel, s->plan, err)) return set_err(ZR_ERR_MODEL, err);
        int ndev = 0;
        if (hipGetDeviceCount(&ndev) != hipSuccess || device < 0 || device >= ndev) {
            (void)hipGetLastError();
            return set_err(ZR_ERR_DEVICE, "no HIP device " + std::to_string(device));
        }
        HIP_TRY(hipSetDevice(device));
        const size_t wb = s->plan.weights.size() * sizeof(float);
        HIP_TRY(hipMalloc((void **)&s->weights, wb ? wb : 4));
        HIP_TRY(hipMemcpy(s->weights, s->plan.weights.data(), wb, hipMemcpyHostToDevice));
        *out = s.release();
        return ZR_OK;
    });
}

void zr_session_destroy(zr_session *s) { delete s; }

int zr_session_num_io(const zr_session *s, int is_output, size_t *n) {
    return guarded([&]() -> int {
        if (int rc = check_session(s)) return rc;
        if (!n) return set_err(ZR_ERR_INVALID_ARGUMENT, "null n");
        *n = is_output ? s->plan.outputs.size() : 1;
        return ZR_OK;
    });
}

int zr_session_io(const zr_session *s, int is_output, size_t idx, const char **name,
                  int64_t *shape, size_t *rank) {
    return guarded([&]() -> int {
        if (int rc = check_session(s)) return rc;
        if (!is_output) {
            if (idx != 0) return set_err(ZR_ERR_INVALID_ARGUMENT, "input index out of range");
            if (name) *name = s->plan.input_name.c_str();
            if (shape) {
                shape[0] = 1;
                shape[1] = s->plan.in_C;
                shape[2] = s->plan.in_H;
                shape[3] = s->plan.in_W;
            }
            if (rank) *rank = 4;
            return ZR_OK;
        }
        if (idx >= s->plan.outputs.size()) return set_err(ZR_ERR_INVALID_ARGUMENT, "output index out of range");
        const auto &o = s->plan.outputs[idx];
        if (name) *name = o.name.c_str();
        if (shape)
            for (size_t i = 0; i < o.shape.size() && i < 8; i++) shape[i] = i == 0 ? 1 : o.shape[i];
        if (rank) *rank = o.shape.size();
        return ZR_OK;
    });
}

int zr_plan_describe(const uint8_t *onnx, size_t len, const uint32_t *out_sel, size_t n_sel,
                     char *buf, size_t cap, size_t *needed) {
    return guarded([&]() -> int {
        if (!onnx) return set_err(ZR_ERR_INVALID_ARGUMENT, "null model");
        zr::OnnxModel m;
        std::string err;
        if (!zr::parse_onnx(onnx, len, m, err)) return set_err(ZR_ERR_MODEL, "ONNX parse error: " + err);
        zr::Plan plan;
        std::vector<uint32_t> sel(out_sel, out_sel + n_sel);
        if (!zr::compile_plan(m, sel, plan, err)) return set_err(ZR_ERR_MODEL, err);
        static const char *kinds[] = {"gemm", "dw", "direct", "elt", "resize", "gap", "dwpw", "dwgap", "gdc"};
        static const char *acts[] = {"none", "relu", "clip", "prelu", "sigmoid"};
        std::string t;
        char line[512];
        auto ref = [](const zr::TRef &r) {
            char b[96];
            snprintf(b, sizeof b, "%s%d[%dx%dx%d]", r.kind == 0 ? "t" : r.kind == 1 ? "in" : "out",
                     r.id, r.C, r.H, r.W);
            return std::string(b);
        };
        snprintf(line, sizeof line, "input %s %dx%dx%d arena_per_image=%lld weights=%zu bytes/img=%.0f flops/img=%.0f fusable=%d\n",
                 plan.input_name.c_str(), plan.in_C, plan.in_H, plan.in_W,
                 (long long)plan.arena_per_image, plan.weights.size(), plan.bytes_per_image,
                 plan.flops_per_image, plan.input_fusable ? 1 : 0);
        t += line;
        for (auto &o : plan.outputs) {
            snprintf(line, sizeof line, "output %s per_image=%lld\n", o.name.c_str(), (long long)o.per_image);
            t += line;
        }
        for (auto &st : plan.steps) {
            snprintf(line, sizeof line,
                     "%s%s in=%s out=%s k=%dx%d s=%d M=%d K=%d KK=%d pre=%s post=%s res=%d rC=%d elt=%d off=%lld oN=%lld oC=%lld oP=%lld in2=%s grp=%d ir=%d%s\n",
                     kinds[st.kind], st.stem ? " stem" : "", ref(st.in).c_str(), ref(st.out).c_str(), st.kh, st.kw, st.stride,
                     st.M, st.K, st.KK, acts[st.pre.kind], acts[st.post.kind], st.res_mode, st.r_C,
                     st.elt_op, (long long)st.out.off, (long long)st.out.o_sN, (long long)st.out.o_sC,
                     (long long)st.out.o_sP, (st.res_mode || st.kind == zr::S_ELT) ? ref(st.in2).c_str() : "-", st.group,
                     st.ir, st.sb ? " sb=1" : "");
            t += line;
        }
        if (needed) *needed = t.size() + 1;
        if (buf && cap) {
            size_t n = std::min(cap - 1, t.size());
            memcpy(buf, t.data(), n);
            buf[n] = 0;
        }
        return ZR_OK;
    });
}

int zr_profile_enable(zr_session *s, int enable) {
    return guarded([&]() -> int {
        if (int rc = check_session(s)) return rc;
        std::lock_guard<std::mutex> g(s->prof.mu);
        s->prof.on = enable != 0;
        return ZR_OK;
    });
}

int zr_profile_read(zr_session *s, char *buf, size_t cap, size_t *needed) {
    return guarded([&]() -> int {
        if (int rc = check_session(s)) return rc;
        std::lock_guard<std::mutex> g(s->prof.mu);
        struct Agg {
            size_t n = 0;
            double ms = 0, bytes = 0, flops = 0;
        };
        std::vector<std::pair<std::string, Agg>> aggs;
        for (auto &r : s->prof.recs) {
            HIP_TRY(hipEventSynchronize(r.b));
            float ms = 0.f;
            HIP_TRY(hipEventElapsedTime(&ms, r.a, r.b));
            auto it = std::find_if(aggs.begin(), aggs.end(), [&](auto &p) { return p.first == r.kernel; });
            if (it == aggs.end()) {
                aggs.push_back({r.kernel, Agg{}});
                it = aggs.end() - 1;
            }
            it->second.n++;
            it->second.ms += ms;
            it->second.bytes += r.bytes;
            it->second.flops += r.flops;
            s->prof.pool.push_back(r.a);
            s->prof.pool.push_back(r.b);
        }
        s->prof.recs.clear();
        std::string t;
        char line[256];
        for (auto &a : aggs) {
            snprintf(line, sizeof line, "%s %zu %.6f %.0f %.0f\n", a.first.c_str(), a.second.n, a.second.ms,
                     a.second.bytes, a.second.flops);
            t += line;
        }
        if (needed) *needed = t.size() + 1;
        if (buf && cap) {
            size_t n = std::min(cap - 1, t.size());
            memcpy(buf, t.data(), n);
            buf[n] = 0;
        }
        return ZR_OK;
    });
}

int zr_session_stats(const zr_session *s, double *bytes, double *flops, size_t *launches) {
    return guarded([&]() -> int {
        if (int rc = check_session(s)) return rc;
        if (bytes) *bytes = s->plan.bytes_per_image;
        if (flops) *flops = s->plan.flops_per_image;
        if (launches) *launches = s->plan.steps.size();
        return ZR_OK;
    });
}

int zr_session_run_async(zr_session *s, size_t batch, const float *d_input, float *const *d_outputs,
                         size_t n_out, void *hip_stream) {
    return guarded([&]() -> int {
        if (int rc = check_session(s)) return rc;
        if (!d_input || !d_outputs || batch == 0) return set_err(ZR_ERR_INVALID_ARGUMENT, "null tensor or empty batch");
        if (n_out != s->plan.outputs.size()) return set_err(ZR_ERR_SHAPE, "output count mismatch");
        Ctx *c = s->acquire();
        if (!c) return set_err(ZR_ERR_DEVICE, "cannot create execution context");
        CtxLock lk(c);
        HIP_TRY(hipSetDevice(s->device));
        const int64_t hw = (int64_t)s->plan.in_H * s->plan.in_W;
        return enqueue(s, c, (int)batch, d_input, hw * s->plan.in_C, hw, d_outputs,
                       (hipStream_t)hip_stream);
    });
}

int zr_session_run(zr_session *s, size_t batch, const float *const *inputs, size_t n_in,
                   float *const *outputs, size_t n_out) {
    return guarded([&]() -> int {
        if (int rc = check_session(s)) return rc;
        if (!inputs || !outputs || batch == 0) return set_err(ZR_ERR_INVALID_ARGUMENT, "null tensor or empty batch");
        if (n_in != 1) return set_err(ZR_ERR_SHAPE, "CNN sessions take exactly 1 input");
        if (n_out != s->plan.outputs.size()) return set_err(ZR_ERR_SHAPE, "output count mismatch");
        Ctx *c = s->acquire();
        if (!c) return set_err(ZR_ERR_DEVICE, "cannot create execution context");
        CtxLock lk(c);
        HIP_TRY(hipSetDevice(s->device));
        const int64_t hw = (int64_t)s->plan.in_H * s->plan.in_W;
        const size_t in_floats = (size_t)hw * s->plan.in_C * batch;
        if (int rc = ctx_stream(c)) return rc;
        if (int rc = grow(c->input, c->input_floats, in_floats)) return rc;
        if (int rc = sync_outputs(s, c, batch)) return rc;
        HIP_TRY(hipMemcpyAsync(c->input, inputs[0], in_floats * 4, hipMemcpyHostToDevice, c->stream));
        if (int rc = enqueue(s, c, (int)batch, c->input, hw * s->plan.in_C, hw, c->outs.data(), c->stream))
            return rc;
        for (size_t i = 0; i < n_out; i++)
            HIP_TRY(hipMemcpyAsync(outputs[i], c->outs[i], s->plan.outputs[i].per_image * batch * 4,
                                   hipMemcpyDeviceToHost, c->stream));
        HIP_TRY(hipStreamSynchronize(c->stream));
        return ZR_OK;
    });
}

static int views_common(zr_session *s, Ctx *c, const zr_frame *frames, size_t nf, const zr_view *views,
                        const uint32_t *view_frame, size_t nv, float lo, float hi, float *const *outs,
                        hipStream_t stream, const zr::ViewDesc *d_views = nullptr, const int *d_nact = nullptr) {
    const int64_t hw = (int64_t)s->plan.in_H * s->plan.in_W;
    if (s->plan.in_C != 3) return set_err(ZR_ERR_SHAPE, "view sampling needs a 3-channel input");
    if (!(hi > lo)) return set_err(ZR_ERR_INVALID_ARGUMENT, "ColorMapper range must satisfy end > start");
    HIP_TRY(hipStreamWaitEvent(stream, c->done, 0));
    if (int rc = upload_views(c, frames, nf, views, view_frame, d_views ? 0 : nv, stream)) return rc;
    zr::PreprocParams p{};
    p.frames = c->frames;
    p.nframes = (int)nf;
    p.views = d_views ? d_views : c->views;
    p.nviews = (int)nv;
    p.OW = s->plan.in_W;
    p.OH = s->plan.in_H;
    p.lo = lo;
    p.adjust = (hi - lo) / 255.0f;
    if (s->plan.input_fusable)
        return enqueue(s, c, (int)nv, nullptr, 0, 0, outs, stream, &p, d_nact);
    if (int rc = grow(c->input, c->input_floats, (size_t)hw * 3 * nv)) return rc;
    p.out = c->input;
    p.o_sN = hw;
    p.o_sC = hw * (int64_t)nv;
    {
        const bool prof = s->prof.on.load();
        std::unique_lock<std::mutex> pl(s->prof.mu, std::defer_lock);
        if (prof) pl.lock();
        if (prof) s->prof.before(stream);
        const char *k = zr::launch_preproc(p, stream);
        if (prof) s->prof.after(stream, k, 16.0 * (double)hw * nv, 0.0);
    }
    HIP_TRY(hipGetLastError());
    return enqueue(s, c, (int)nv, c->input, hw, hw * (int64_t)nv, outs, stream, nullptr, d_nact);
}

int zr_cnn_estimate_views_async(zr_session *s, const zr_frame *frames, size_t n_frames,
                                const zr_view *views, const uint32_t *view_frame, size_t n_views,
                                float lo, float hi, float *const *d_outputs, void *hip_stream) {
    return guarded([&]() -> int {
        if (int rc = check_session(s)) return rc;
        if (!frames || !views || !d_outputs || n_views == 0)
            return set_err(ZR_ERR_INVALID_ARGUMENT, "null argument or no views");
        Ctx *c = s->acquire();
        if (!c) return set_err(ZR_ERR_DEVICE, "cannot create execution context");
        CtxLock lk(c);
        HIP_TRY(hipSetDevice(s->device));
        return views_common(s, c, frames, n_frames, views, view_frame, n_views, lo, hi, d_outputs,
                            (hipStream_t)hip_stream);
    });
}

static_assert(sizeof(zr_track_state) == sizeof(zr::TrackState), "zr_track_state layout");
static_assert(sizeof(zr_view_desc) == sizeof(zr::ViewDesc), "zr_view_desc layout");

static int check_track_cfg(const zr_track_cfg *cfg, size_t n) {
    if (!cfg || n == 0) return set_err(ZR_ERR_INVALID_ARGUMENT, "null argument or n == 0");
    if (cfg->kind < 0 || cfg->kind > 3 || cfg->num_landmarks <= 0 || cfg->in_w <= 0 || cfg->in_h <= 0 ||
        cfg->aspect_w <= 0 || cfg->aspect_h <= 0 || !(cfg->padding >= 0.f) || n > (1u << 24))
        return set_err(ZR_ERR_INVALID_ARGUMENT, "bad tracker configuration");
    if ((cfg->kind == 0 && cfg->num_landmarks <= 263) || (cfg->kind == 1 && cfg->num_landmarks <= 9))
        return set_err(ZR_ERR_INVALID_ARGUMENT, "angle landmarks out of range");
    return ZR_OK;
}

static int check_extract_inputs(const zr_track_cfg *cfg, const float *d_landmarks, size_t lm_stride,
                                const float *d_flag, size_t flag_stride) {
    if (!d_landmarks || (cfg->kind <= 2 && (!d_flag || flag_stride == 0)))
        return set_err(ZR_ERR_INVALID_ARGUMENT, "missing landmark / flag outputs");
    if (flag_stride > (size_t)INT32_MAX) return set_err(ZR_ERR_INVALID_ARGUMENT, "flag stride too large");
    if (cfg->kind == 2 && (cfg->num_landmarks <= 5 || flag_stride < 15))
        return set_err(ZR_ERR_INVALID_ARGUMENT, "eye network: output 1 holds the 5 iris points");
    const size_t L = (size_t)cfg->num_landmarks;
    const size_t need = cfg->kind == 3 ? 2 * L : cfg->kind == 2 ? 3 * (L - 5) : 3 * L;
    if (lm_stride < need || lm_stride > (size_t)INT32_MAX)
        return set_err(ZR_ERR_SHAPE, "landmark output holds fewer floats per image than the extract reads");
    return ZR_OK;
}

static int track_params(zr::TrackParams &p, zr_track_state *d_state, size_t n, const zr_track_cfg *cfg,
                        zr_view_desc *d_views) {
    if (!d_state || !cfg || !d_views || n == 0) return set_err(ZR_ERR_INVALID_ARGUMENT, "null argument or n == 0");
    if (int rc = check_track_cfg(cfg, n)) return rc;
    p.state = reinterpret_cast<zr::TrackState *>(d_state);
    p.views = reinterpret_cast<zr::ViewDesc *>(d_views);
    p.n = (int)n;
    p.L = cfg->num_landmarks;
    p.kind = cfg->kind;
    p.in_w = cfg->in_w;
    p.in_h = cfg->in_h;
    p.asp_w = cfg->aspect_w;
    p.asp_h = cfg->aspect_h;
    p.loss_thresh = cfg->loss_thresh;
    p.padding = cfg->padding;
    if (cfg->rois_per_frame < 0) return set_err(ZR_ERR_INVALID_ARGUMENT, "rois_per_frame must be >= 0");
    p.rpf = cfg->rois_per_frame > 0 ? cfg->rois_per_frame : 1;
    return ZR_OK;
}

int zr_track_seed_async(zr_track_state *d_state, size_t n, const zr_track_cfg *cfg, zr_view_desc *d_views,
                        void *hip_stream) {
    return guarded([&]() -> int {
        zr::TrackParams p{};
        if (int rc = track_params(p, d_state, n, cfg, d_views)) return rc;
        p.seed = 1;
        zr::launch_track(p, (hipStream_t)hip_stream);
        HIP_TRY(hipGetLastError());
        return ZR_OK;
    });
}

static int track_update(zr_track_state *d_state, size_t n, const zr_track_cfg *cfg, const float *d_landmarks,
                        size_t lm_stride, const float *d_flag, size_t flag_stride, const int32_t *d_index,
                        float *d_lm_out, zr_view_desc *d_views, void *hip_stream) {
    return guarded([&]() -> int {
        zr::TrackParams p{};
        if (int rc = track_params(p, d_state, n, cfg, d_views)) return rc;
        if (int rc = check_extract_inputs(cfg, d_landmarks, lm_stride, d_flag, flag_stride)) return rc;
        p.lm = d_landmarks;
        p.lm_stride = (int)lm_stride;
        p.flag = d_flag;
        p.flag_stride = (int)flag_stride;
        p.index = d_index;
        p.lm_out = d_lm_out;
        zr::launch_track(p, (hipStream_t)hip_stream);
        HIP_TRY(hipGetLastError());
        return ZR_OK;
    });
}

int zr_track_update_async(zr_track_state *d_state, size_t n, const zr_track_cfg *cfg, const float *d_landmarks,
                          size_t lm_stride, const float *d_flag, size_t flag_stride, float *d_lm_out,
                          zr_view_desc *d_views, void *hip_stream) {
    return track_update(d_state, n, cfg, d_landmarks, lm_stride, d_flag, flag_stride, nullptr, d_lm_out, d_views,
                        hip_stream);
}

int zr_track_update_indexed_async(zr_track_state *d_state, size_t n, const zr_track_cfg *cfg,
                                  const float *d_landmarks, size_t lm_stride, const float *d_flag,
                                  size_t flag_stride, const int32_t *d_index, float *d_lm_out,
                                  zr_view_desc *d_views, void *hip_stream) {
    return track_update(d_state, n, cfg, d_landmarks, lm_stride, d_flag, flag_stride, d_index, d_lm_out, d_views,
                        hip_stream);
}

static int track_update_positions(zr_track_state *d_state, size_t n, const zr_track_cfg *cfg,
                                  const float *d_positions, const float *d_flag, size_t flag_stride,
                                  const int32_t *d_index, float *d_lm_out, zr_view_desc *d_views, void *hip_stream) {
    return guarded([&]() -> int {
        zr::TrackParams p{};
        if (int rc = track_params(p, d_state, n, cfg, d_views)) return rc;
        if (!d_positions) return set_err(ZR_ERR_INVALID_ARGUMENT, "missing positions");
        if (cfg->kind <= 1 && (!d_flag || flag_stride == 0 || flag_stride > (size_t)INT32_MAX))
            return set_err(ZR_ERR_INVALID_ARGUMENT, "missing flag output");
        p.pos = d_positions;
        if (cfg->kind <= 1) {
            p.flag = d_flag;
            p.flag_stride = (int)flag_stride;
        }
        p.index = d_index;
        p.lm_out = d_lm_out;
        zr::launch_track(p, (hipStream_t)hip_stream);
        HIP_TRY(hipGetLastError());
        return ZR_OK;
// ... 846 lines not shown
        p.lm = d_eye_lm;
        p.diam = d_eye_diam;
        p.valid = d_eye_valid;
        p.n = (int)n;
        p.in_w = cfg->in_w;
        p.asp_w = cfg->aspect_w;
        p.asp_h = cfg->aspect_h;
        zr::launch_eye_commit(p, (hipStream_t)hip_stream);
        HIP_TRY(hipGetLastError());
        return ZR_OK;
    });
}

static_assert(sizeof(zr_export_header) == sizeof(zr::ExportHeader) && sizeof(zr_export_header) == 48,
              "zr_export_header layout");
static_assert(offsetof(zr_export_header, flags) == offsetof(zr::ExportHeader, flags), "zr_export_header layout");
static_assert(sizeof(zr_export_identity) == sizeof(zr::ExportIdentity) && sizeof(zr_export_identity) == 16,
              "zr_export_identity layout");
static_assert(sizeof(zr_pose) == 4 * zr::EXPORT_POSE_WORDS, "zr_pose words");
static_assert(3 * ZR_EYE_POINTS == zr::EXPORT_EYE_WORDS, "eye landmark words");
static_assert(ZR_EXPORT_POSE == zr::EXPORT_POSE && ZR_EXPORT_IDENTITY == zr::EXPORT_IDENTITY &&
                  ZR_EXPORT_EYE_LEFT == zr::EXPORT_EYE_LEFT && ZR_EXPORT_EYE_RIGHT == zr::EXPORT_EYE_RIGHT &&
                  ZR_EXPORT_QUALITY == zr::EXPORT_QUALITY,
              "export flags");
static_assert(sizeof(zr_face_quality) == 4 * zr::EXPORT_QUALITY_WORDS, "zr_face_quality words");

static int multi_export(const zr_multi_export_args *a, const zr_face_quality *d_quality, zr_face_quality *d_out_quality,
                        size_t n_streams, size_t slots, size_t num_landmarks, void *hip_stream) {
    return guarded([&]() -> int {
        if (!a) return set_err(ZR_ERR_INVALID_ARGUMENT, "null argument");
        if (!a->d_nobjects || !a->d_src || !a->d_ids || !a->d_roi || !a->d_state || !a->d_landmarks || !a->d_count ||
            !a->d_stream_offsets || !a->d_header || !a->d_out_landmarks)
            return set_err(ZR_ERR_INVALID_ARGUMENT, "null argument");
        const int pose = (a->d_pose != nullptr) + (a->d_out_pose != nullptr);
        const int ident = (a->d_id_state != nullptr) + (a->d_id_emb != nullptr) + (a->d_out_identity != nullptr) +
                          (a->d_out_emb != nullptr);
        const int eyes = (a->d_eye_valid != nullptr) + (a->d_eye_diam != nullptr) + (a->d_eye_crop != nullptr) +
                         (a->d_eye_lm != nullptr) + (a->d_out_eye_valid != nullptr) + (a->d_out_eye_diam != nullptr) +
                         (a->d_out_eye_crop != nullptr) + (a->d_out_eye_lm != nullptr);
        const int qual = (d_quality != nullptr) + (d_out_quality != nullptr);
        if ((pose != 0 && pose != 2) || (ident != 0 && ident != 4) || (eyes != 0 && eyes != 8) || (qual != 0 && qual != 2))
            return set_err(ZR_ERR_INVALID_ARGUMENT,
                           "an optional group (pose, identity, eyes, quality) is given in full or not at all");
        if (n_streams == 0) return set_err(ZR_ERR_INVALID_ARGUMENT, "no streams");
        if (slots == 0 || slots > 64) return set_err(ZR_ERR_INVALID_ARGUMENT, "slots must be 1..64");
        if (num_landmarks == 0 || num_landmarks > (1u << 20))
            return set_err(ZR_ERR_INVALID_ARGUMENT, "num_landmarks must be 1..2^20");
        if (n_streams > (size_t)INT32_MAX / slots)
            return set_err(ZR_ERR_INVALID_ARGUMENT, "streams x slots beyond the kernel's 32-bit record index");
        zr::ExportParams p{};
        p.nobjects = a->d_nobjects;
        p.src = a->d_src;
        p.ids = a->d_ids;
        p.roi = a->d_roi;
        p.state = reinterpret_cast<const zr::TrackState *>(a->d_state);
        p.lm = reinterpret_cast<const uint32_t *>(a->d_landmarks);
        p.pose = reinterpret_cast<const uint32_t *>(a->d_pose);
        p.ist = reinterpret_cast<const zr::IdentityState *>(a->d_id_state);
        p.emb = reinterpret_cast<const uint32_t *>(a->d_id_emb);
        p.eye_valid = a->d_eye_valid;
        p.eye_diam = reinterpret_cast<const uint32_t *>(a->d_eye_diam);
        p.eye_crop = reinterpret_cast<const uint32_t *>(a->d_eye_crop);
        p.eye_lm = reinterpret_cast<const uint32_t *>(a->d_eye_lm);
        p.quality = reinterpret_cast<const uint32_t *>(d_quality);
        p.count = a->d_count;
        p.offsets = a->d_stream_offsets;
        p.header = reinterpret_cast<zr::ExportHeader *>(a->d_header);
        p.out_lm = reinterpret_cast<uint32_t *>(a->d_out_landmarks);
        p.out_pose = reinterpret_cast<uint32_t *>(a->d_out_pose);
        p.out_ist = reinterpret_cast<zr::ExportIdentity *>(a->d_out_identity);
        p.out_emb = reinterpret_cast<uint32_t *>(a->d_out_emb);
        p.out_eye_valid = a->d_out_eye_valid;
        p.out_eye_diam = reinterpret_cast<uint32_t *>(a->d_out_eye_diam);
        p.out_eye_crop = reinterpret_cast<uint32_t *>(a->d_out_eye_crop);
        p.out_eye_lm = reinterpret_cast<uint32_t *>(a->d_out_eye_lm);
        p.out_quality = reinterpret_cast<uint32_t *>(d_out_quality);
        p.S = (int)n_streams;
        p.K = (int)slots;
        p.L = (int)num_landmarks;
        const uintptr_t bases = (uintptr_t)a->d_landmarks | (uintptr_t)a->d_out_landmarks | (uintptr_t)a->d_id_emb |
                                (uintptr_t)a->d_out_emb | (uintptr_t)a->d_eye_lm | (uintptr_t)a->d_out_eye_lm;
        p.vec4 = (3 * num_landmarks) % 4 == 0 && bases % 16 == 0 ? 1 : 0;
        zr::launch_export(p, (hipStream_t)hip_stream);
        HIP_TRY(hipGetLastError());
        return ZR_OK;
    });
}

int zr_multi_export_async(const zr_multi_export_args *a, size_t n_streams, size_t slots, size_t num_landmarks,
                          void *hip_stream) {
    return multi_export(a, nullptr, nullptr, n_streams, slots, num_landmarks, hip_stream);
}

int zr_multi_export_quality_async(const zr_multi_export_args *a, const zr_face_quality *d_quality,
                                  zr_face_quality *d_out_quality, size_t n_streams, size_t slots,
                                  size_t num_landmarks, void *hip_stream) {
    return multi_export(a, d_quality, d_out_quality, n_streams, slots, num_landmarks, hip_stream);
}

int zr_view_describe(const zr_view *views, size_t n, uint32_t frame, zr_view_desc *out) {
    return guarded([&]() -> int {
        if (!views || !out) return set_err(ZR_ERR_INVALID_ARGUMENT, "null argument");
        for (size_t i = 0; i < n; i++) {
            const zr::ViewDesc d = make_view(views[i], frame);
            std::memcpy(&out[i], &d, sizeof(d));
        }
        return ZR_OK;
    });
}

int zr_debug_glibc_math(int fn, const float *d_a, const float *d_b, float *d_out, size_t n, void *hip_stream) {
    return guarded([&]() -> int {
        if (fn < 0 || fn > 4 || !d_a || !d_out || (fn == 4 && !d_b) || n > (size_t)INT64_MAX / 2)
            return set_err(ZR_ERR_INVALID_ARGUMENT, "bad glibc-math request");
        if (n == 0) return ZR_OK;
        zr::launch_glibc_math(fn, d_a, d_b, d_out, (int64_t)n, (hipStream_t)hip_stream);
        HIP_TRY(hipGetLastError());
        return ZR_OK;
    });
}

int zr_cnn_estimate_device_views_async(zr_session *s, const zr_frame *frames, size_t n_frames,
                                       const zr_view_desc *d_views, size_t n_views, float lo, float hi,
                                       float *const *d_outputs, void *hip_stream) {
    return guarded([&]() -> int {
        if (int rc = check_session(s)) return rc;
        if (!frames || !d_views || !d_outputs || n_views == 0 || n_frames == 0)
            return set_err(ZR_ERR_INVALID_ARGUMENT, "null argument or no views");
        Ctx *c = s->acquire();
        if (!c) return set_err(ZR_ERR_DEVICE, "cannot create execution context");
        CtxLock lk(c);
        HIP_TRY(hipSetDevice(s->device));
        return views_common(s, c, frames, n_frames, nullptr, nullptr, n_views, lo, hi, d_outputs,
                            (hipStream_t)hip_stream, reinterpret_cast<const zr::ViewDesc *>(d_views));
    });
}

int zr_cnn_estimate_device_views_count_async(zr_session *s, const zr_frame *frames, size_t n_frames,
                                             const zr_view_desc *d_views, size_t n_views, const int32_t *d_count,
                                             float lo, float hi, float *const *d_outputs, void *hip_stream) {
    return guarded([&]() -> int {
        if (int rc = check_session(s)) return rc;
        if (!frames || !d_views || !d_outputs || !d_count || n_views == 0 || n_frames == 0)
            return set_err(ZR_ERR_INVALID_ARGUMENT, "null argument or no views");
        Ctx *c = s->acquire();
        if (!c) return set_err(ZR_ERR_DEVICE, "cannot create execution context");
        CtxLock lk(c);
        HIP_TRY(hipSetDevice(s->device));
        return views_common(s, c, frames, n_frames, nullptr, nullptr, n_views, lo, hi, d_outputs,
                            (hipStream_t)hip_stream, reinterpret_cast<const zr::ViewDesc *>(d_views), d_count);
    });
}

int zr_due_compact_async(const int32_t *d_det_pending, size_t n, const zr_view_desc *view_template, int32_t *d_due,
                         int32_t *d_ndue, zr_view_desc *d_due_views, uint64_t *d_total, void *hip_stream) {
    return guarded([&]() -> int {
        if (!d_det_pending || !view_template || !d_due || !d_ndue || !d_due_views)
            return set_err(ZR_ERR_INVALID_ARGUMENT, "null argument");
        if (n == 0 || n > (1u << 24)) return set_err(ZR_ERR_INVALID_ARGUMENT, "bad stream count");
        zr::launch_due_compact(d_det_pending, nullptr, (int)n, *reinterpret_cast<const zr::ViewDesc *>(view_template),
                               d_due, d_ndue, reinterpret_cast<zr::ViewDesc *>(d_due_views), d_total,
                               (hipStream_t)hip_stream);
        HIP_TRY(hipGetLastError());
        return ZR_OK;
    });
}

int zr_due_compact_tiles_async(const int32_t *d_det_pending, size_t n, const zr_view_desc *d_tile_templates,
                               size_t tiles, int32_t *d_due, int32_t *d_ndue, int32_t *d_due_slots,
                               zr_view_desc *d_due_views, int32_t *d_nviews, uint64_t *d_total_streams,
                               uint64_t *d_total_views, void *hip_stream) {
    return guarded([&]() -> int {
        if (!d_det_pending || !d_tile_templates || !d_due || !d_ndue || !d_due_slots || !d_due_views || !d_nviews)
            return set_err(ZR_ERR_INVALID_ARGUMENT, "null argument");
        if (n == 0 || n > (1u << 24)) return set_err(ZR_ERR_INVALID_ARGUMENT, "bad stream count");
        if (tiles < 1 || tiles > 16) return set_err(ZR_ERR_INVALID_ARGUMENT, "tiles must be 1..16");
        zr::DueTilesParams p{};
        p.pending = d_det_pending;
        p.tmpl = reinterpret_cast<const zr::ViewDesc *>(d_tile_templates);
        p.S = (int)n;
        p.T = (int)tiles;
        p.due = d_due;
        p.ndue = d_ndue;
        p.due_slots = d_due_slots;
        p.due_views = reinterpret_cast<zr::ViewDesc *>(d_due_views);
        p.nviews = d_nviews;
        p.total_streams = d_total_streams;
        p.total_views = d_total_views;
        zr::launch_due_compact_tiles(p, (hipStream_t)hip_stream);
        HIP_TRY(hipGetLastError());
        return ZR_OK;
    });
}

int zr_detect_merge_async(const int32_t *d_tile_count, const float *d_tile_dets, const int32_t *d_due,
                          const int32_t *d_ndue, size_t n, const zr_detmerge_cfg *cfg, int32_t *d_count,
                          float *d_dets, size_t dcap, int32_t *d_ties, int32_t *d_tile_dropped, void *hip_stream) {
    return guarded([&]() -> int {
        if (!d_tile_count || !d_tile_dets || !d_due || !d_ndue || !cfg || !d_count || !d_dets)
            return set_err(ZR_ERR_INVALID_ARGUMENT, "null argument");
        if (n == 0 || n > (1u << 24)) return set_err(ZR_ERR_INVALID_ARGUMENT, "bad stream count");
        if (cfg->tiles < 1 || cfg->tiles > 16 || cfg->tile_cap < 1 || cfg->tile_cap > 256 ||
            cfg->tiles * cfg->tile_cap > 1024 || cfg->keypoints < 0 || cfg->keypoints > 7 || dcap == 0 ||
            dcap > 65536 || cfg->mode < 0 || cfg->mode > 1)
            return set_err(ZR_ERR_INVALID_ARGUMENT, "bad detection merge configuration");
        zr::DetMergeParams p{};
        p.tile_count = d_tile_count;
        p.tile_dets = d_tile_dets;
        p.due = d_due;
        p.ndue = d_ndue;
        p.S = (int)n;
        p.T = cfg->tiles;
        p.tile_cap = cfg->tile_cap;
        p.nkp = cfg->keypoints;
        p.iou = cfg->iou;
        p.mode = cfg->mode;
        p.count = d_count;
        p.dets = d_dets;
        p.dcap = (int)dcap;
        p.ties = d_ties;
        p.tile_dropped = d_tile_dropped;
        zr::launch_det_merge(p, (hipStream_t)hip_stream);
        HIP_TRY(hipGetLastError());
        return ZR_OK;
    });
}

int zr_track_lost_compact_async(const zr_track_state *d_state, size_t n, const zr_view_desc *view_template,
                                int32_t *d_due, int32_t *d_ndue, zr_view_desc *d_due_views, uint64_t *d_total,
                                void *hip_stream) {
    return guarded([&]() -> int {
        if (!d_state || !view_template || !d_due || !d_ndue || !d_due_views)
            return set_err(ZR_ERR_INVALID_ARGUMENT, "null argument");
        if (n == 0 || n > (1u << 24)) return set_err(ZR_ERR_INVALID_ARGUMENT, "bad stream count");
        zr::launch_due_compact(nullptr, reinterpret_cast<const zr::TrackState *>(d_state), (int)n,
                               *reinterpret_cast<const zr::ViewDesc *>(view_template), d_due, d_ndue,
                               reinterpret_cast<zr::ViewDesc *>(d_due_views), d_total, (hipStream_t)hip_stream);
        HIP_TRY(hipGetLastError());
        return ZR_OK;
    });
}

int zr_track_reseed_best_async(const int32_t *d_count, const float *d_dets, size_t dcap, const uint32_t *d_frame_size,
                               size_t n, const zr_track_cfg *cfg, zr_track_state *d_state, zr_view_desc *d_views,
                               uint64_t *d_reseeded, void *hip_stream) {
    return guarded([&]() -> int {
        if (!d_count || !d_dets || !d_frame_size || !cfg || !d_state || !d_views || dcap == 0)
            return set_err(ZR_ERR_INVALID_ARGUMENT, "null argument");
        if (n == 0) return ZR_OK;
        if (cfg->aspect_w <= 0 || cfg->aspect_h <= 0 || n > (1u << 24) || dcap > 65536)
            return set_err(ZR_ERR_INVALID_ARGUMENT, "bad re-seeding configuration");
        zr::ReseedParams p{};
        p.count = d_count;
        p.dets = d_dets;
        p.dcap = (int)dcap;
        p.fsize = d_frame_size;
        p.N = (int)n;
        p.asp_w = cfg->aspect_w;
        p.asp_h = cfg->aspect_h;
        p.state = reinterpret_cast<zr::TrackState *>(d_state);
        p.views = reinterpret_cast<zr::ViewDesc *>(d_views);
        p.reseeded = d_reseeded;
        zr::launch_reseed(p, (hipStream_t)hip_stream);
        HIP_TRY(hipGetLastError());
        return ZR_OK;
    });
}

int zr_cnn_estimate_views(zr_session *s, const uint8_t *rgba, uint32_t w, uint32_t h,
                          size_t row_stride, const zr_view *views, size_t n_views, float lo,
                          float hi, float *const *outputs) {
    return guarded([&]() -> int {
        if (int rc = check_session(s)) return rc;
        if (!rgba || !views || !outputs || n_views == 0)
            return set_err(ZR_ERR_INVALID_ARGUMENT, "null argument or no views");
        if (row_stride < (size_t)w * 4) return set_err(ZR_ERR_INVALID_ARGUMENT, "row_stride < 4*width");
        Ctx *c = s->acquire();
        if (!c) return set_err(ZR_ERR_DEVICE, "cannot create execution context");
        CtxLock lk(c);
        HIP_TRY(hipSetDevice(s->device));
        const size_t bytes = row_stride * h;
        if (int rc = ctx_stream(c)) return rc;
        if (int rc = grow(c->image, c->image_bytes, bytes ? bytes : 4)) return rc;
        if (int rc = sync_outputs(s, c, n_views)) return rc;
        HIP_TRY(hipStreamWaitEvent(c->stream, c->done, 0));
        HIP_TRY(hipMemcpyAsync(c->image, rgba, bytes, hipMemcpyHostToDevice, c->stream));
        zr_frame f{c->image, w, h, (uint64_t)row_stride};
        if (int rc = views_common(s, c, &f, 1, views, nullptr, n_views, lo, hi, c->outs.data(), c->stream))
            return rc;
        for (size_t i = 0; i < s->plan.outputs.size(); i++)
            HIP_TRY(hipMemcpyAsync(outputs[i], c->outs[i], s->plan.outputs[i].per_image * n_views * 4,
                                   hipMemcpyDeviceToHost, c->stream));
        HIP_TRY(hipStreamSynchronize(c->stream));
        return ZR_OK;
    });
}

int zr_preprocess_views_async(const zr_frame *frames, size_t n_frames, const zr_view *views,
                              const uint32_t *view_frame, size_t n_views, uint32_t ow, uint32_t oh,
                              float lo, float hi, float *d_out, void *hip_stream) {
    return guarded([&]() -> int {
        if (!frames || !views || !d_out || n_views == 0 || ow == 0 || oh == 0)
            return set_err(ZR_ERR_INVALID_ARGUMENT, "null argument or empty shape");
        if (!(hi > lo)) return set_err(ZR_ERR_INVALID_ARGUMENT, "ColorMapper range must satisfy end > start");
        hipStream_t st = (hipStream_t)hip_stream;
        std::vector<zr::ViewDesc> vd(n_views);
// ... 278 lines not shown
```

Before: 275,800.

## Split detect and landmark stages onto separate streams with resident view tables

```diff
diff --git a/include/zaru_hip.h b/include/zaru_hip.h
--- a/include/zaru_hip.h
+++ b/include/zaru_hip.h
@@ -217,6 +217,18 @@
 int zr_cnn_estimate_device_views_count_async(zr_session *s, const zr_frame *frames, size_t n_frames,
                                              const zr_view_desc *d_views, size_t n_views, const int32_t *d_count,
                                              float lo, float hi, float *const *d_outputs, void *hip_stream);
+typedef struct {
+    const uint8_t *rgba;
+    uint32_t w, h;
+    uint64_t stride;
+} zr_frame_desc;
+int zr_views_upload_async(const zr_frame *frames, size_t n_frames, const zr_view *views, const uint32_t *view_frame,
+                          size_t n_views, void *h_staging, size_t staging_bytes, zr_frame_desc *d_frames,
+                          zr_view_desc *d_views, void *hip_stream);
+int zr_cnn_estimate_resident_async(zr_session *s, const zr_frame_desc *d_frames, size_t n_frames,
+                                   const zr_view_desc *d_views, size_t n_views, float lo, float hi,
+                                   float *const *d_outputs, void *hip_stream);
+int zr_session_max_views(const zr_session *s, size_t *n);
 int zr_due_compact_async(const int32_t *d_det_pending, size_t n, const zr_view_desc *view_template, int32_t *d_due,
                          int32_t *d_ndue, zr_view_desc *d_due_views, uint64_t *d_total, void *hip_stream);
 int zr_due_compact_tiles_async(const int32_t *d_det_pending, size_t n, const zr_view_desc *d_tile_templates,
diff --git a/zaru_amd/_lib.py b/zaru_amd/_lib.py
--- a/zaru_amd/_lib.py
+++ b/zaru_amd/_lib.py
@@ -227,6 +227,9 @@
     ("zr_comm_all_gather_async", _I, [_P, _P, _P, _SZ, _P]),
     ("zr_debug_glibc_math", _I, [_I, _P, _P, _P, _SZ, _P]),
     ("zr_cnn_estimate_device_views_async", _I, [_P, _P, _SZ, _P, _SZ, _F, _F, _P, _P]),
+    ("zr_views_upload_async", _I, [_P, _SZ, _P, _P, _SZ, _P, _SZ, _P, _P, _P]),
+    ("zr_cnn_estimate_resident_async", _I, [_P, _P, _SZ, _P, _SZ, _F, _F, _P, _P]),
+    ("zr_session_max_views", _I, [_P, C.POINTER(_SZ)]),
     ("zr_jpeg_decoder_create", _I, [C.c_int, _P]),
     ("zr_jpeg_decoder_destroy", None, [_P]),
     ("zr_jpeg_info", _I, [_P, _SZ, _P, _P]),
diff --git a/zaru_amd/csrc/host/bindings.cpp b/zaru_amd/csrc/host/bindings.cpp
--- a/zaru_amd/csrc/host/bindings.cpp
+++ b/zaru_amd/csrc/host/bindings.cpp
@@ -894,11 +894,27 @@
         .def("detections_run", &DeviceFaceLoop::detections_run)
         .def("reacquisitions", &DeviceFaceLoop::reacquisitions);
 
+    m.def("pipeline_schedule", [](uint32_t sub_batches, size_t n_frames, bool device_post, bool stream_per_sub_batch,
+                                  bool stage_streams, size_t max_images_per_launch, uint32_t rois_per_frame) {
+        const PipelineSchedule sch = pipeline_schedule(sub_batches, n_frames, device_post, stream_per_sub_batch,
+                                                       stage_streams, max_images_per_launch, rois_per_frame);
+        py::list ranges;
+        for (const auto &r : sch.ranges) ranges.append(py::make_tuple(r.f0, r.nf, r.det_stream, r.lm_stream));
+        py::dict d;
+        d["ranges"] = ranges;
+        d["stage_streams"] = sch.stage_streams;
+        d["streams"] = sch.streams;
+        return d;
+    }, py::arg("sub_batches"), py::arg("n_frames"), py::arg("device_post") = true,
+       py::arg("stream_per_sub_batch") = true, py::arg("stage_streams") = true,
+       py::arg("max_images_per_launch") = 0, py::arg("rois_per_frame") = 1);
+
     py::class_<DetectTrackPipeline>(m, "DetectTrackPipeline")
         .def(py::init([](const std::string &kind, int device, int threads, uint32_t max_rois,
                          uint32_t sub_batches, bool stream_per_sub_batch, float loss_threshold,
                          const std::string &detector, const std::string &landmarker, bool device_post,
-                         const std::string &nms_mode, uint32_t det_cap, float det_threshold) {
+                         const std::string &nms_mode, uint32_t det_cap, float det_threshold,
+                         py::object stage_streams) {
                  PipelineConfig c = kind == "hand" ? PipelineConfig::hand() : PipelineConfig::face();
                  if (kind != "hand" && kind != "face")
                      throw ZaruError(ZR_ERR_INVALID_ARGUMENT, "pipeline kind must be 'face' or 'hand'");
@@ -913,6 +929,7 @@
                  else if (nms_mode != "average") throw ZaruError(ZR_ERR_INVALID_ARGUMENT, "nms_mode: average | remove");
                  c.det_cap = det_cap;
                  c.det_threshold = det_threshold;
+                 if (!stage_streams.is_none()) c.stage_streams = stage_streams.cast<bool>();
                  return new DetectTrackPipeline(c, device, threads);
              }), py::arg("kind") = "face", py::arg("device") = 0, py::arg("threads") = 8,
              py::arg("max_rois_per_frame") = 8, py::arg("sub_batches") = 2,
@@ -920,7 +937,7 @@
              py::arg("loss_threshold") = LandmarkTracker::DEFAULT_LOSS_THRESHOLD,
              py::arg("detector") = "", py::arg("landmarker") = "", py::arg("device_post") = true,
              py::arg("nms_mode") = "average", py::arg("det_cap") = 0,
-             py::arg("det_threshold") = Detector::DEFAULT_THRESHOLD)
+             py::arg("det_threshold") = Detector::DEFAULT_THRESHOLD, py::arg("stage_streams") = py::none())
         .def("run", [](DetectTrackPipeline &p, const std::vector<std::tuple<uint64_t, uint32_t, uint32_t, uint64_t>> &frames,
                        const std::vector<std::vector<std::tuple<float, float, float, float, float>>> &forced) {
             std::vector<Image> im;
@@ -1037,6 +1054,8 @@
             d["map_ms"] = t.map_ms;
             d["total_ms"] = t.total_ms;
             d["host_wait_ms"] = t.host_wait_ms;
+            d["step_gap_ms"] = t.step_gap_ms;
+            d["step_gaps"] = t.step_gaps;
             d["dropped_detections"] = t.dropped_detections;
             d["nms_candidates"] = t.nms_candidates;
             d["nms_tied"] = t.nms_tied;
diff --git a/zaru_amd/csrc/host/pipeline.cpp b/zaru_amd/csrc/host/pipeline.cpp
--- a/zaru_amd/csrc/host/pipeline.cpp
+++ b/zaru_amd/csrc/host/pipeline.cpp
@@ -2,6 +2,7 @@
 
 #include <algorithm>
 #include <condition_variable>
+#include <cstdlib>
 #include <cstring>
 #include <mutex>
 
@@ -111,36 +112,115 @@
         check(zr_memcpy_async(d_anchors_.ptr, a.data(), a.size() * sizeof(Vec2), 0, nullptr));
         check(zr_stream_synchronize(nullptr));
     }
-    check(zr_stream_create(&stream_));
-    for (uint32_t i = 0; i < std::max(1u, cfg_.sub_batches); i++) {
+    if (const char *e = std::getenv("ZARU_PIPELINE_SCHEDULE")) {
+        const std::string v(e);
+        if (v == "stage") cfg_.stage_streams = true;
+        else if (v == "ahead" || v == "drain") cfg_.stage_streams = false;
+        else if (!v.empty()) throw ZaruError(ZR_ERR_INVALID_ARGUMENT, "ZARU_PIPELINE_SCHEDULE: stage | ahead | drain");
+        drain_ = v == "drain";
+    }
+    const uint32_t ns = pipeline_schedule(cfg_.sub_batches, 0, cfg_.device_post, cfg_.stream_per_sub_batch,
+                                          cfg_.stage_streams).streams;
+    for (uint32_t i = 0; i < ns; i++) {
+        void *st = nullptr;
+        check(zr_stream_create(&st));
+        streams_.push_back(st);
+    }
+    stream_ = streams_[0];
+    size_t md = 0, ml = 0;
+    check(zr_session_max_views(det_cnn_->nn().handle(), &md));
+    check(zr_session_max_views(lm_cnn_->nn().handle(), &ml));
+    max_launch_ = std::min(md, ml);
+}
+
+DetectTrackPipeline::Slot &DetectTrackPipeline::slot(size_t k) {
+    while (slots_.size() <= k) {
         slots_.push_back(std::make_unique<Slot>());
         Slot &s = *slots_.back();
-        if (cfg_.stream_per_sub_batch && i > 0) check(zr_stream_create(&s.stream));
-        else s.stream = stream_;
         check(zr_event_create(&s.ev_det));
         check(zr_event_create(&s.ev_lm));
         check(zr_event_create(&s.ev_rec));
-        for (auto &e : s.ev_t) check(zr_event_create_timing(&e));
-    }
+        for (auto &e : s.ev_end) check(zr_event_create_timing(&e));
+        for (auto &o : s.res) {
+            check(zr_event_create(&o.ev_lm));
+            for (auto &e : o.ev_t) check(zr_event_create_timing(&e));
+        }
+    }
+    return *slots_[k];
 }
 
 DetectTrackPipeline::~DetectTrackPipeline() {
+    for (void *st : streams_) zr_stream_synchronize(st);
+    if (gstream_) {
+        zr_stream_synchronize(gstream_);
+        zr_stream_destroy(gstream_);
+    }
     for (auto &s : slots_) {
-        if (s->stream) zr_stream_synchronize(s->stream);
-        if (s->stream && s->stream != stream_) zr_stream_destroy(s->stream);
         if (s->ev_det) zr_event_destroy(s->ev_det);
         if (s->ev_lm) zr_event_destroy(s->ev_lm);
         if (s->ev_rec) zr_event_destroy(s->ev_rec);
-        for (auto e : s->ev_t)
+        for (auto e : s->ev_end)
             if (e) zr_event_destroy(e);
-    }
-    if (gstream_) {
-        zr_stream_synchronize(gstream_);
-        zr_stream_destroy(gstream_);
+        for (auto &o : s->res) {
+            if (o.ev_lm) zr_event_destroy(o.ev_lm);
+            for (auto e : o.ev_t)
+                if (e) zr_event_destroy(e);
+        }
     }
     for (auto e : ev_gath_)
         if (e) zr_event_destroy(e);
-    if (stream_) zr_stream_destroy(stream_);
+    for (void *st : streams_) zr_stream_destroy(st);
+}
+
+PipelineSchedule pipeline_schedule(uint32_t sub_batches, size_t n_frames, bool device_post, bool stream_per_sub_batch,
+                                   bool stage_streams, size_t max_images_per_launch, uint32_t rois_per_frame) {
+    PipelineSchedule sch;
+    const size_t S = std::max(1u, sub_batches);
+    sch.stage_streams = stage_streams && device_post && stream_per_sub_batch && S >= 2;
+    const size_t pairs = S / 2;
+    sch.streams = (uint32_t)(sch.stage_streams ? 2 * pairs : stream_per_sub_batch ? S : 1);
+    if (n_frames == 0) return sch;
+    size_t R = std::min(sch.stage_streams ? pairs : S, n_frames);
+    if (max_images_per_launch > 0) {
+        const size_t per = std::max<size_t>(1, max_images_per_launch / std::max(1u, rois_per_frame));
+        R = std::max(R, (n_frames + per - 1) / per);
+    }
+    size_t f0 = 0;
+    for (size_t k = 0; k < R; k++) {
+        PipelineSchedule::Range r;
+        r.f0 = f0;
+        r.nf = n_frames / R + (k < n_frames % R ? 1 : 0);
+        f0 += r.nf;
+        if (sch.stage_streams) {
+            r.det_stream = (uint32_t)(2 * (k % pairs));
+            r.lm_stream = r.det_stream + 1;
+        } else {
+            r.det_stream = r.lm_stream = (uint32_t)(stream_per_sub_batch ? k % S : 0);
+        }
+        sch.ranges.push_back(r);
+    }
+    return sch;
+}
+
+void DetectTrackPipeline::assign_ranges(size_t n_frames) {
+    for (auto &sp : slots_) {
+        for (; sp->fin < sp->enq; sp->fin++) check(zr_event_synchronize(sp->res[sp->fin & 1].ev_lm));
+        sp->chained = false;
+    }
+    const PipelineSchedule sch =
+        pipeline_schedule(cfg_.sub_batches, n_frames, cfg_.device_post, cfg_.stream_per_sub_batch, cfg_.stage_streams,
+                          max_launch_, std::max(1u, cfg_.max_rois_per_frame));
+    for (size_t k = 0; k < sch.ranges.size(); k++) {
+        const PipelineSchedule::Range &r = sch.ranges[k];
+        Slot &s = slot(k);
+        void *ds = streams_[r.det_stream], *ls = streams_[r.lm_stream];
+        if (s.f0 != r.f0 || s.nf != r.nf || s.stream != ds || s.lm_stream != ls) s.inputs_ok = false;
+        s.f0 = r.f0;
+        s.nf = r.nf;
+        s.stream = ds;
+        s.lm_stream = ls;
+    }
+    active_slots_ = sch.ranges.size();
 }
 
 size_t DetectTrackPipeline::det_cap() const { return cfg_.det_cap; }
@@ -256,6 +336,18 @@
     const uint32_t A = (uint32_t)cfg_.detector.anchors().size(), D = (uint32_t)cfg_.detector.params;
     const uint32_t cap = cfg_.candidate_cap, rec_w = 2 + D;
     const size_t n = s.nf;
+    s.d_boxes.resize(n * A * D);
+    s.d_logits.resize(n * A);
+    float *douts[2] = {s.d_boxes.ptr, s.d_logits.ptr};
+    if (cfg_.device_post) {
+        Slot::Results &o = s.res[s.enq & 1];
+        const ColorMapper cm = dc.color_mapper();
+        check(zr_event_record(o.ev_t[0], s.stream));
+        check(zr_cnn_estimate_resident_async(dc.nn().handle(), s.d_frames.ptr, n, s.d_detviews.ptr, n, cm.lo, cm.hi,
+                                             douts, s.stream));
+        check(zr_event_record(o.ev_t[1], s.stream));
+        return;
+    }
     s.zf.resize(n);
     s.letterbox.resize(n);
     std::vector<zr_view> zv(n);
@@ -267,17 +359,9 @@
         zv[i] = to_zr_view(letterbox_view(im.width, im.height, dc.aspect(), &s.letterbox[i]));
         vf[i] = (uint32_t)i;
     }
-    s.d_boxes.resize(n * A * D);
-    s.d_logits.resize(n * A);
     s.d_count.resize(n);
     s.d_rec.resize(n * cap * rec_w);
-    float *douts[2] = {s.d_boxes.ptr, s.d_logits.ptr};
-    if (cfg_.device_post) check(zr_event_record(s.ev_t[0], s.stream));
     dc.estimate_async(s.zf, zv, vf, douts, s.stream);
-    if (cfg_.device_post) {
-        check(zr_event_record(s.ev_t[1], s.stream));
-        return;
-    }
     check(zr_detection_candidates_async(s.d_logits.ptr, s.d_boxes.ptr, (uint32_t)n, A, D,
                                         candidate_logit_floor(cfg_.det_threshold), cap, s.d_count.ptr,
                                         s.d_rec.ptr, s.stream));
@@ -303,14 +387,37 @@
     return c;
 }
 
-void DetectTrackPipeline::stage_device_post(Slot &s, const std::vector<Image> &frames,
-                                            const std::vector<std::vector<RotatedRect>> &forced) {
-    const Cnn &dc = *det_cnn_, &lc = *lm_cnn_;
-    const size_t n = s.nf, R = std::max(1u, cfg_.max_rois_per_frame), dcap = cfg_.det_cap;
-    const size_t nv = n * R, nout = lc.nn().num_outputs();
-    const int L = cfg_.landmarker.num_landmarks;
-    const uint32_t A = (uint32_t)cfg_.detector.anchors().size(), D = (uint32_t)cfg_.detector.params;
-    if (!s.inputs_ok) {
+void DetectTrackPipeline::enqueue_device_step(Slot &s, const std::vector<Image> &frames,
+                                              const std::vector<std::vector<RotatedRect>> &forced) {
+    prepare_device_inputs(s, frames, forced);
+    stage_detect(s, frames);
+    stage_device_post(s, frames, forced);
+}
+
+void DetectTrackPipeline::prepare_device_inputs(Slot &s, const std::vector<Image> &frames,
+                                                const std::vector<std::vector<RotatedRect>> &forced) {
+    if (s.inputs_ok) return;
+    const Cnn &dc = *det_cnn_;
+    const size_t n = s.nf, R = std::max(1u, cfg_.max_rois_per_frame), nv = n * R;
+    {
+        s.zf.resize(n);
+        s.letterbox.resize(n);
+        std::vector<zr_view> zv(n);
+        std::vector<uint32_t> vf(n);
+        for (size_t i = 0; i < n; i++) {
+            const Image &im = frames[s.f0 + i];
+            if (!im.on_device) throw ZaruError(ZR_ERR_INVALID_ARGUMENT, "pipeline frames must be device-resident");
+            s.zf[i] = zr_frame{im.rgba, im.width, im.height, im.row_stride};
+            zv[i] = to_zr_view(letterbox_view(im.width, im.height, dc.aspect(), &s.letterbox[i]));
+            vf[i] = (uint32_t)i;
+        }
+        check(zr_stream_synchronize(s.stream));
+        const size_t bytes = n * (sizeof(zr_view_desc) + sizeof(zr_frame_desc));
+        s.h_desc.resize(bytes);
+        s.d_frames.resize(n);
+        s.d_detviews.resize(n);
+        check(zr_views_upload_async(s.zf.data(), n, zv.data(), vf.data(), n, s.h_desc.ptr, bytes, s.d_frames.ptr,
+                                    s.d_detviews.ptr, s.stream));
         s.h_lbox.resize(4 * n);
         s.h_fsize.resize(2 * n);
         s.h_forced.resize(5 * nv);
@@ -346,7 +453,17 @@
         check(zr_memcpy_async(s.d_nforced.ptr, s.h_nforced.ptr, n * 4, 0, s.stream));
         s.inputs_ok = true;
     }
-    Slot::Results &o = s.res[s.wr];
+}
+
+void DetectTrackPipeline::stage_device_post(Slot &s, const std::vector<Image> &frames,
+                                            const std::vector<std::vector<RotatedRect>> &forced) {
+    const Cnn &dc = *det_cnn_, &lc = *lm_cnn_;
+    const size_t n = s.nf, R = std::max(1u, cfg_.max_rois_per_frame), dcap = cfg_.det_cap;
+    const size_t nv = n * R, nout = lc.nn().num_outputs();
+    const int L = cfg_.landmarker.num_landmarks;
+    const uint32_t A = (uint32_t)cfg_.detector.anchors().size(), D = (uint32_t)cfg_.detector.params;
+    (void)forced;
+    Slot::Results &o = s.res[s.enq & 1];
     const size_t sum_bytes = 2 * nv * sizeof(zr_track_state) + 3 * n * sizeof(int32_t);
     o.sum.resize(sum_bytes);
     o.h_sum.resize(sum_bytes);
@@ -356,7 +473,7 @@
     zr_track_state *d_seed = d_state + nv;
     int32_t *d_count = reinterpret_cast<int32_t *>(d_seed + nv);
     int32_t *d_ties = d_count + n;
-    s.d_views.resize(nv);
+    o.views.resize(nv);
     zr_detpost_cfg pc{};
     pc.face = is_face_detector(cfg_.detector.kind) ? 1 : 0;
     pc.anchors = (int)A;
@@ -382,31 +499,44 @@
     const zr_track_cfg tc = track_cfg();
     check(zr_track_seed_detections_async(d_count, o.dets.ptr, dcap, s.d_forced.ptr, s.d_nforced.ptr, s.d_fsize.ptr,
                                          n, &tc, cfg_.roi_grow, cfg_.roi_use_angle ? 1 : 0, d_state, d_seed,
-                                         s.d_views.ptr, s.stream));
-    check(zr_event_record(s.ev_t[2], s.stream));
+                                         o.views.ptr, s.stream));
+    check(zr_event_record(o.ev_t[2], s.stream));
+    void *ls = s.lm_stream;
+    if (ls != s.stream) {
+        check(zr_stream_wait_event(ls, o.ev_t[2]));
+        check(zr_event_record(o.ev_t[4], ls));
+    }
     float *lptr[4] = {nullptr, nullptr, nullptr, nullptr};
     for (size_t k = 0; k < nout && k < 4; k++) {
         o.lm[k].resize((size_t)lc.nn().output_per_image(k) * nv);
         lptr[k] = o.lm[k].ptr;
     }
     const ColorMapper cm = lc.color_mapper();
-    check(zr_cnn_estimate_device_views_async(lc.nn().handle(), s.zf.data(), n, s.d_views.ptr, nv, cm.lo, cm.hi, lptr,
-                                             s.stream));
-    check(zr_event_record(s.ev_t[3], s.stream));
+    check(zr_cnn_estimate_resident_async(lc.nn().handle(), s.d_frames.ptr, n, o.views.ptr, nv, cm.lo, cm.hi, lptr, ls));
+    check(zr_event_record(o.ev_t[3], ls));
     const bool flagged = tc.kind <= 2;
     check(zr_track_update_async(d_state, nv, &tc, lptr[0], (size_t)lc.nn().output_per_image(0),
                                 flagged ? lptr[1] : nullptr, flagged ? (size_t)lc.nn().output_per_image(1) : 0,
-                                o.lmout.ptr, s.d_views.ptr, s.stream));
-    check(zr_event_record(s.ev_t[4], s.stream));
-    check(zr_memcpy_async(o.h_sum.ptr, o.sum.ptr, sum_bytes, 1, s.stream));
-    check(zr_event_record(s.ev_lm, s.stream));
-    s.timed = true;
-    s.wr ^= 1;
+                                o.lmout.ptr, o.views.ptr, ls));
+    o.ev_end = s.ev_end[s.enq % 3];
+    check(zr_event_record(o.ev_end, ls));
+    check(zr_memcpy_async(o.h_sum.ptr, o.sum.ptr, sum_bytes, 1, ls));
+    check(zr_event_record(o.ev_lm, ls));
+    o.timed = true;
+    s.enq++;
+}
+
+void DetectTrackPipeline::wait_device_step(Slot &s) {
+    if (s.fin == s.enq) throw ZaruError(ZR_ERR_INVALID_ARGUMENT, "step() without a begun sequence");
+    const auto t = clk::now();
+    check(zr_event_synchronize(s.res[s.fin & 1].ev_lm));
+    times_.host_wait_ms += ms_since(t);
+    finish_device(s);
 }
 
 void DetectTrackPipeline::finish_device(Slot &s) {
-    s.done = s.wr ^ 1;
-    const Slot::Results &o = s.res[s.done];
+    s.done = (int)(s.fin & 1);
+    Slot::Results &o = s.res[s.done];
     const size_t n = s.nf, R = std::max(1u, cfg_.max_rois_per_frame), nv = n * R;
     const zr_track_state *st = reinterpret_cast<const zr_track_state *>(o.h_sum.ptr);
     const int32_t *cnt = reinterpret_cast<const int32_t *>(st + 2 * nv), *tie = cnt + n;
@@ -415,15 +545,27 @@
         times_.detections += (size_t)cnt[i];
         if ((size_t)cnt[i] > cfg_.det_cap) times_.dropped_detections += (size_t)cnt[i] - cfg_.det_cap;
     }
-    if (s.timed) {
+    if (o.timed) {
         float ms[4] = {0.f, 0.f, 0.f, 0.f};
-        for (int k = 0; k < 4; k++) check(zr_event_elapsed(&ms[k], s.ev_t[k], s.ev_t[k + 1]));
+        check(zr_event_elapsed(&ms[0], o.ev_t[0], o.ev_t[1]));
+        check(zr_event_elapsed(&ms[1], o.ev_t[1], o.ev_t[2]));
+        check(zr_event_elapsed(&ms[2], o.ev_t[s.lm_stream != s.stream ? 4 : 2], o.ev_t[3]));
+        check(zr_event_elapsed(&ms[3], o.ev_t[3], o.ev_end));
         times_.detect_gpu_ms += ms[0];
         times_.decode_nms_ms += ms[1];
         times_.landmark_gpu_ms += ms[2];
         times_.map_ms += ms[3];
-        s.timed = false;
-    }
+        if (s.chained) {
+            float gap = 0.f;
+            if (zr_event_elapsed(&gap, s.ev_end[(s.fin + 2) % 3], o.ev_t[0]) == ZR_OK) {
+                times_.step_gap_ms += gap;
+                times_.step_gaps++;
+            }
+        }
+        o.timed = false;
+    }
+    s.fin++;
+    s.chained = true;
     for (size_t v = 0; v < nv; v++) {
         times_.rois += st[nv + v].active ? 1 : 0;
         times_.tracked += st[v].tracked ? 1 : 0;
@@ -629,28 +771,22 @@
     ties_.assign(B, {});
     rois_.clear();
     if (B == 0) return;
-    const size_t S = std::min<size_t>(slots_.size(), B);
-    size_t f0 = 0;
+    const bool resident = &frames == &frames_ && &forced == &forced_;
+    if (!resident)
+        for (auto &s : slots_) s->inputs_ok = false;
+    assign_ranges(B);
+    const size_t S = active_slots_;
     for (size_t k = 0; k < S; k++) {
         Slot &s = *slots_[k];
-        s.f0 = f0;
-        s.nf = B / S + (k < B % S ? 1 : 0);
-        f0 += s.nf;
-        s.inputs_ok = false;
-        stage_detect(s, frames);
-        if (cfg_.device_post) stage_device_post(s, frames, forced);
-    }
-    active_slots_ = S;
+        if (cfg_.device_post) enqueue_device_step(s, frames, forced);
+        else stage_detect(s, frames);
+    }
     if (cfg_.device_post && rec_rmax_ && &frames == &frames_) enqueue_gather();
-    for (size_t k = 0; k < S && cfg_.device_post; k++) {
-        Slot &s = *slots_[k];
-        const auto t = clk::now();
-        check(zr_event_synchronize(s.ev_lm));
-        times_.host_wait_ms += ms_since(t);
-        finish_device(s);
-    }
+    for (size_t k = 0; k < S && cfg_.device_post; k++) wait_device_step(*slots_[k]);
     if (cfg_.device_post) done_steps_ = enq_steps_;
     if (cfg_.device_post) {
+        if (!resident)
+            for (auto &s : slots_) s->inputs_ok = false;
         times_.total_ms = ms_since(t0);
         return;
     }
@@ -686,17 +822,11 @@
     enq_steps_ = done_steps_ = 0;
     gath_used_[0] = gath_used_[1] = false;
     const std::vector<Image> &frames = frames_;
-    const size_t B = frames.size();
-    active_slots_ = std::min<size_t>(slots_.size(), B);
-    size_t f0 = 0;
+    assign_ranges(frames.size());
     for (size_t k = 0; k < active_slots_; k++) {
         Slot &s = *slots_[k];
-        s.f0 = f0;
-        s.nf = B / active_slots_ + (k < B % active_slots_ ? 1 : 0);
-        f0 += s.nf;
-        s.inputs_ok = false;
-        stage_detect(s, frames);
-        if (cfg_.device_post) stage_device_post(s, frames, forced_);
+        if (cfg_.device_post) enqueue_device_step(s, frames, forced_);
+        else stage_detect(s, frames);
     }
     if (cfg_.device_post) enqueue_gather();
 }
@@ -708,20 +838,17 @@
     dets_.assign(B, {});
     ties_.assign(B, {});
     rois_.clear();
+    if (cfg_.device_post && more && !drain_) {
+        for (size_t k = 0; k < S; k++) enqueue_device_step(*slots_[k], frames, forced_);
+        enqueue_gather();
+    }
     for (size_t k = 0; k < S && cfg_.device_post; k++) {
-        Slot &s = *slots_[k];
-        const auto t = clk::now();
-        check(zr_event_synchronize(s.ev_lm));
-        times_.host_wait_ms += ms_since(t);
-        finish_device(s);
-        if (more) {
-            stage_detect(s, frames);
-            stage_device_post(s, frames, forced_);
-        }
+        wait_device_step(*slots_[k]);
+        if (more && drain_) enqueue_device_step(*slots_[k], frames, forced_);
     }
     if (cfg_.device_post) {
         done_steps_++;
-        if (more) enqueue_gather();
+        if (more && drain_) enqueue_gather();
         times_.frames += B;
         times_.total_ms = ms_since(steps_t0_);
         return;
diff --git a/zaru_amd/csrc/host/pipeline.h b/zaru_amd/csrc/host/pipeline.h
--- a/zaru_amd/csrc/host/pipeline.h
+++ b/zaru_amd/csrc/host/pipeline.h
@@ -38,6 +38,8 @@
 struct StageTimes {
     double detect_gpu_ms = 0, decode_nms_ms = 0, landmark_gpu_ms = 0, map_ms = 0, total_ms = 0;
     double host_wait_ms = 0;
+    double step_gap_ms = 0;
+    size_t step_gaps = 0;
     size_t frames = 0, detections = 0, rois = 0, tracked = 0;
     size_t dropped_detections = 0;
     size_t nms_candidates = 0, nms_tied = 0, nms_unpinned_frames = 0;
@@ -59,9 +61,23 @@
     bool stream_per_sub_batch = true;
     bool device_post = true;
     uint32_t det_cap = 0;
+    bool stage_streams = false;
     static PipelineConfig face();
     static PipelineConfig hand();
 };
+
+struct PipelineSchedule {
+    struct Range {
+        size_t f0, nf;
+        uint32_t det_stream, lm_stream;
+    };
+    std::vector<Range> ranges;
+    bool stage_streams = false;
+    uint32_t streams = 1;
+};
+PipelineSchedule pipeline_schedule(uint32_t sub_batches, size_t n_frames, bool device_post, bool stream_per_sub_batch,
+                                   bool stage_streams, size_t max_images_per_launch = 0,
+                                   uint32_t rois_per_frame = 1);
 
 class DetectTrackPipeline {
   public:
@@ -103,11 +119,9 @@
   private:
     struct Slot {
         size_t f0 = 0, nf = 0;
-        void *stream = nullptr;
+        void *stream = nullptr, *lm_stream = nullptr;
         void *ev_det = nullptr, *ev_lm = nullptr;
-        void *ev_t[5] = {nullptr, nullptr, nullptr, nullptr, nullptr};
         void *ev_rec = nullptr;
-        bool timed = false;
         DeviceArray<float> d_boxes, d_logits, d_rec, d_lm[4];
         DeviceArray<int32_t> d_count;
         PinnedArray<float> h_rec, h_lm[4];
@@ -120,19 +134,35 @@
         DeviceArray<float> d_lbox, d_forced;
         DeviceArray<uint32_t> d_fsize;
         DeviceArray<int32_t> d_nforced;
-        DeviceArray<zr_view_desc> d_views;
         PinnedArray<float> h_lbox, h_forced;
         PinnedArray<uint32_t> h_fsize;
         PinnedArray<int32_t> h_nforced;
+        DeviceArray<zr_frame_desc> d_frames;
+        DeviceArray<zr_view_desc> d_detviews;
+        PinnedArray<uint8_t> h_desc;
         bool inputs_ok = false;
         struct Results {
             DeviceArray<uint8_t> sum;
             DeviceArray<float> dets, lmout, lm[4];
+            DeviceArray<zr_view_desc> views;
             PinnedArray<uint8_t> h_sum;
+            void *ev_lm = nullptr;
+            void *ev_t[5] = {nullptr, nullptr, nullptr, nullptr, nullptr};
+            void *ev_end = nullptr;
+            bool timed = false;
         } res[2];
-        int wr = 0;
+        uint64_t enq = 0, fin = 0;
+        void *ev_end[3] = {nullptr, nullptr, nullptr};
         int done = 0;
+        bool chained = false;
     };
+    Slot &slot(size_t k);
+    void assign_ranges(size_t n_frames);
+    void prepare_device_inputs(Slot &s, const std::vector<Image> &frames,
+                               const std::vector<std::vector<RotatedRect>> &forced);
+    void enqueue_device_step(Slot &s, const std::vector<Image> &frames,
+                             const std::vector<std::vector<RotatedRect>> &forced);
+    void wait_device_step(Slot &s);
     void stage_device_post(Slot &s, const std::vector<Image> &frames,
                            const std::vector<std::vector<RotatedRect>> &forced);
     void finish_device(Slot &s);
@@ -153,6 +183,9 @@
     NonMaxSuppression nms_;
     ThreadPool pool_;
     void *stream_ = nullptr;
+    std::vector<void *> streams_;
+    bool drain_ = false;
+    size_t max_launch_ = 0;
     std::vector<std::unique_ptr<Slot>> slots_;
     mutable std::vector<std::vector<Detection>> dets_;
     std::vector<NonMaxSuppression::TieCount> ties_;
diff --git a/zaru_amd/csrc/runtime/session.cpp b/zaru_amd/csrc/runtime/session.cpp
--- a/zaru_amd/csrc/runtime/session.cpp
+++ b/zaru_amd/csrc/runtime/session.cpp
@@ -262,14 +262,18 @@
     }
 };
 
+size_t largest_tensor(const zr::Plan &plan, size_t N, size_t in_sN) {
+    size_t largest = std::max((size_t)plan.arena_per_image * ((N + 3) / 4 * 4), in_sN * N);
+    for (const auto &o : plan.outputs) largest = std::max(largest, (size_t)o.per_image * N);
+    return largest;
+}
+
 int enqueue(zr_session *s, Ctx *c, int N, const float *input, int64_t in_sN, int64_t in_sC,
             float *const *outs, hipStream_t stream, const zr::PreprocParams *pre = nullptr,
             const int *d_nact = nullptr) {
     const int Ns = (N + 3) / 4 * 4;
     const size_t need = (size_t)s->plan.arena_per_image * (size_t)Ns;
-    size_t largest = std::max(need, (size_t)(input ? in_sN : 0) * (size_t)N);
-    for (const auto &o : s->plan.outputs) largest = std::max(largest, (size_t)o.per_image * (size_t)N);
-    if (largest >= ((size_t)1 << 31))
+    if (largest_tensor(s->plan, (size_t)N, input ? (size_t)in_sN : 0) >= ((size_t)1 << 31))
         return set_err(ZR_ERR_INVALID_ARGUMENT, "batch too large: a tensor would exceed 2^31 elements; split it");
     if (int rc = grow(c->arena, c->arena_floats, need ? need : 1)) return rc;
     HIP_TRY(hipStreamWaitEvent(stream, c->done, 0));
@@ -315,6 +319,24 @@
     return ZR_OK;
 }
 
+int fill_tables(const zr_frame *frames, size_t nf, const zr_view *views, const uint32_t *view_frame, size_t nv,
+                zr::ViewDesc *hv, zr::FrameDesc *hf) {
+    for (size_t i = 0; i < nv; i++) {
+        const uint32_t f = view_frame ? view_frame[i] : 0;
+        if (f >= nf) return set_err(ZR_ERR_INVALID_ARGUMENT, "view_frame index out of range");
+        hv[i] = make_view(views[i], f);
+    }
+    for (size_t i = 0; i < nf; i++) {
+        if (!frames[i].rgba || frames[i].width == 0 || frames[i].height == 0)
+            return set_err(ZR_ERR_INVALID_ARGUMENT, "empty frame");
+        hf[i].rgba = frames[i].rgba;
+        hf[i].w = frames[i].width;
+        hf[i].h = frames[i].height;
+        hf[i].stride = frames[i].row_stride;
+    }
+    return ZR_OK;
+}
+
 int upload_views(Ctx *c, const zr_frame *frames, size_t nf, const zr_view *views,
                  const uint32_t *view_frame, size_t nv, hipStream_t stream) {
     const size_t foff = (nv * sizeof(zr::ViewDesc) + 255) & ~(size_t)255;
@@ -333,19 +355,7 @@
     zr::FrameDesc *hf = reinterpret_cast<zr::FrameDesc *>(c->h_desc + foff);
     c->views = reinterpret_cast<zr::ViewDesc *>(c->desc);
     c->frames = reinterpret_cast<zr::FrameDesc *>(c->desc + foff);
-    for (size_t i = 0; i < nv; i++) {
-        const uint32_t f = view_frame ? view_frame[i] : 0;
-        if (f >= nf) return set_err(ZR_ERR_INVALID_ARGUMENT, "view_frame index out of range");
-        hv[i] = make_view(views[i], f);
-    }
-    for (size_t i = 0; i < nf; i++) {
-        if (!frames[i].rgba || frames[i].width == 0 || frames[i].height == 0)
-            return set_err(ZR_ERR_INVALID_ARGUMENT, "empty frame");
-        hf[i].rgba = frames[i].rgba;
-        hf[i].w = frames[i].width;
-        hf[i].h = frames[i].height;
-        hf[i].stride = frames[i].row_stride;
-    }
+    if (int rc = fill_tables(frames, nf, views, view_frame, nv, hv, hf)) return rc;
     HIP_TRY(hipMemcpyAsync(c->desc, c->h_desc, foff + nf * sizeof(zr::FrameDesc), hipMemcpyHostToDevice, stream));
     return ZR_OK;
 }
@@ -575,14 +585,16 @@
 
 static int views_common(zr_session *s, Ctx *c, const zr_frame *frames, size_t nf, const zr_view *views,
                         const uint32_t *view_frame, size_t nv, float lo, float hi, float *const *outs,
-                        hipStream_t stream, const zr::ViewDesc *d_views = nullptr, const int *d_nact = nullptr) {
+                        hipStream_t stream, const zr::ViewDesc *d_views = nullptr, const int *d_nact = nullptr,
+                        const zr::FrameDesc *d_frames = nullptr) {
     const int64_t hw = (int64_t)s->plan.in_H * s->plan.in_W;
     if (s->plan.in_C != 3) return set_err(ZR_ERR_SHAPE, "view sampling needs a 3-channel input");
     if (!(hi > lo)) return set_err(ZR_ERR_INVALID_ARGUMENT, "ColorMapper range must satisfy end > start");
     HIP_TRY(hipStreamWaitEvent(stream, c->done, 0));
-    if (int rc = upload_views(c, frames, nf, views, view_frame, d_views ? 0 : nv, stream)) return rc;
+    if (!d_frames)
+        if (int rc = upload_views(c, frames, nf, views, view_frame, d_views ? 0 : nv, stream)) return rc;
     zr::PreprocParams p{};
-    p.frames = c->frames;
+    p.frames = d_frames ? d_frames : c->frames;
     p.nframes = (int)nf;
     p.views = d_views ? d_views : c->views;
     p.nviews = (int)nv;
@@ -1735,6 +1747,60 @@
     });
 }
 
+static_assert(sizeof(zr_frame_desc) == sizeof(zr::FrameDesc), "zr_frame_desc layout");
+
+int zr_views_upload_async(const zr_frame *frames, size_t n_frames, const zr_view *views, const uint32_t *view_frame,
+                          size_t n_views, void *h_staging, size_t staging_bytes, zr_frame_desc *d_frames,
+                          zr_view_desc *d_views, void *hip_stream) {
+    return guarded([&]() -> int {
+        if (!frames || n_frames == 0 || !h_staging || !d_frames || (n_views && (!views || !d_views)))
+            return set_err(ZR_ERR_INVALID_ARGUMENT, "null argument or no frames");
+        const size_t vb = n_views * sizeof(zr::ViewDesc), fb = n_frames * sizeof(zr::FrameDesc);
+        if (staging_bytes < vb + fb) return set_err(ZR_ERR_INVALID_ARGUMENT, "staging buffer too small");
+        uint8_t *h = static_cast<uint8_t *>(h_staging);
+        if (int rc = fill_tables(frames, n_frames, views, view_frame, n_views, reinterpret_cast<zr::ViewDesc *>(h),
+                                 reinterpret_cast<zr::FrameDesc *>(h + vb)))
+            return rc;
+        hipStream_t st = (hipStream_t)hip_stream;
+        if (vb) HIP_TRY(hipMemcpyAsync(d_views, h, vb, hipMemcpyHostToDevice, st));
+        HIP_TRY(hipMemcpyAsync(d_frames, h + vb, fb, hipMemcpyHostToDevice, st));
+        return ZR_OK;
+    });
+}
+
+int zr_cnn_estimate_resident_async(zr_session *s, const zr_frame_desc *d_frames, size_t n_frames,
+                                   const zr_view_desc *d_views, size_t n_views, float lo, float hi,
+                                   float *const *d_outputs, void *hip_stream) {
+    return guarded([&]() -> int {
+        if (int rc = check_session(s)) return rc;
+        if (!d_frames || !d_views || !d_outputs || n_views == 0 || n_frames == 0)
+            return set_err(ZR_ERR_INVALID_ARGUMENT, "null argument or no views");
+        if (n_frames > (size_t)INT32_MAX || n_views > (size_t)INT32_MAX)
+            return set_err(ZR_ERR_INVALID_ARGUMENT, "too many frames or views");
+        Ctx *c = s->acquire();
+        if (!c) return set_err(ZR_ERR_DEVICE, "cannot create execution context");
+        CtxLock lk(c);
+        HIP_TRY(hipSetDevice(s->device));
+        return views_common(s, c, nullptr, n_frames, nullptr, nullptr, n_views, lo, hi, d_outputs,
+                            (hipStream_t)hip_stream, reinterpret_cast<const zr::ViewDesc *>(d_views), nullptr,
+                            reinterpret_cast<const zr::FrameDesc *>(d_frames));
+    });
+}
+
+int zr_session_max_views(const zr_session *s, size_t *n) {
+    return guarded([&]() -> int {
+        if (int rc = check_session(s)) return rc;
+        if (!n) return set_err(ZR_ERR_INVALID_ARGUMENT, "null n");
+        const size_t in_sN = s->plan.input_fusable ? 0 : (size_t)s->plan.in_H * (size_t)s->plan.in_W;
+        const size_t lim = (size_t)1 << 31;
+        size_t N = lim / std::max<size_t>(1, largest_tensor(s->plan, 4, in_sN) / 4);
+        N = std::min<size_t>(N, (size_t)INT32_MAX);
+        while (N > 0 && largest_tensor(s->plan, N, in_sN) >= lim) N--;
+        *n = N;
+        return ZR_OK;
+    });
+}
+
 int zr_due_compact_async(const int32_t *d_det_pending, size_t n, const zr_view_desc *view_template, int32_t *d_due,
                          int32_t *d_ndue, zr_view_desc *d_due_views, uint64_t *d_total, void *hip_stream) {
     return guarded([&]() -> int {
```

Result: no change. 274,800 (-0.4%).
